# nooice98/HM16.9-NN_FME

Measured on AMD Instinct MI355X. Metric: sub-pel PU refinements/sec @ 1080p lowdelay_P QP22; bit-exact MV/SATD vs HM, higher is better.
Workload: dtype int16/int32 (NN f32)

## Files before the change

hm16.9-nn_fme_amd/csrc/fme_api.cpp:

```cpp
#include <dlfcn.h>
#include <hsa/hsa.h>
#include <hsa/hsa_ext_amd.h>

#include <chrono>
#include <cmath>
#include <cstdarg>
#include <cstdio>
#include <memory>

#include "fme_ctx.h"

using namespace fme;

namespace {
thread_local std::string g_last_error = "";
}


int fme::fail(int code, const char* fmt, ...) {
  char buf[512];
  va_list ap;
  va_start(ap, fmt);
  vsnprintf(buf, sizeof(buf), fmt, ap);
  va_end(ap);
  g_last_error = buf;
  return code;
}


extern "C" {

int fme_abi_version(void) { return FME_ABI_VERSION; }

const char* fme_last_error(void) { return g_last_error.c_str(); }

int fme_create(int device, const fme_config* cfg, fme_ctx** out_ctx) {
  if (!cfg || !out_ctx) return fail(FME_E_INVALID, "fme_create: null argument");
  *out_ctx = nullptr;
  if (cfg->bit_depth != 8 && cfg->bit_depth != 10)
    return fail(FME_E_UNSUPPORTED, "fme_create: bit_depth %d (8, or 10 for the main10 configurations)", cfg->bit_depth);
  if (cfg->nn_mode < 0 || cfg->nn_mode > 2) return fail(FME_E_INVALID, "fme_create: nn_mode %d", cfg->nn_mode);
  int ndev = 0;
  HIP_TRY(hipGetDeviceCount(&ndev));
  if (device < 0 || device >= ndev) return fail(FME_E_INVALID, "fme_create: device %d of %d", device, ndev);
  HIP_TRY(hipSetDevice(device));
  std::unique_ptr<fme_ctx> c(new fme_ctx());
  c->device = device;
  c->cfg = *cfg;
  HIP_TRY(c->d_pics.reserve(FME_MAX_PICTURES));
  HIP_TRY(c->d_mlambda.reserve(FME_MAX_LAMBDAS));
  HIP_TRY(c->d_nn.reserve(kNnPkFloats));
  HIP_TRY(c->counts.reserve(2 * kCountWords));
  HIP_TRY(hipMemset(c->counts.p, 0, 2 * kCountWords * sizeof(int32_t)));
  HIP_TRY(c->d_sched.reserve(1));
  c->sched_p = sched_params();
  {
    const char* m10 = std::getenv("FME_MAIN10_SEARCH");
    c->main10_px = m10 && std::strcmp(m10, "px") == 0;
  }
  HIP_TRY(hipEventCreateWithFlags(&c->ev_done, hipEventDisableTiming));
  HIP_TRY(c->nn_state.reserve(24));
  HIP_TRY(hipMemset(c->nn_state.p, 0, 24 * sizeof(uint32_t)));
  HIP_TRY(c->d_key_invalid.reserve(1));
  HIP_TRY(hipMemset(c->d_key_invalid.p, 0, sizeof(int32_t)));
  HIP_TRY(hipHostMalloc(reinterpret_cast<void**>(&c->h_counts), kCountWords * sizeof(int32_t), hipHostMallocDefault));
  if (cfg->max_jobs > 0) {
    const size_t n = (size_t)cfg->max_jobs;
    const size_t nb = (n + kJobsPerScanBlock - 1) / kJobsPerScanBlock;
    if (n * kNumClasses > (size_t)INT32_MAX) return fail(FME_E_INVALID, "fme_create: max_jobs %d", cfg->max_jobs);
    HIP_TRY(c->cls.reserve(n));
    HIP_TRY(c->perm.reserve(n * kNumClasses));
    HIP_TRY(c->blk_agg.reserve(nb * 9));
    HIP_TRY(c->blk_prefix.reserve(nb * 9));
  }
  *out_ctx = c.release();
  return FME_OK;
}

}
static int srv_stop(fme_ctx* c);
static void note_stream(fme_ctx* c, hipStream_t s) {
  for (int i = 0; i < c->n_used_streams; i++)
    if (c->used_streams[i] == s) return;
  if (c->n_used_streams < fme_ctx::kMaxStreams) c->used_streams[c->n_used_streams++] = s;
  else c->used_overflow = true;
}
static int drain_ctx(fme_ctx* c) {
  if (c->used_overflow) {
    HIP_TRY(hipDeviceSynchronize());
  } else {
    for (int i = 0; i < c->n_used_streams; i++) HIP_TRY(hipStreamSynchronize(c->used_streams[i]));
  }
  return FME_OK;
}
int fme::grow_keys(fme_ctx* c, size_t n) {
  if (n <= c->d_keys.cap) return FME_OK;
  FME_TRY(drain_ctx(c));
  HIP_TRY(c->d_keys.reserve(n));
  return FME_OK;
}
extern "C" {
int fme_destroy(fme_ctx* c) {
  if (!c) return FME_OK;
  (void)hipSetDevice(c->device);
  (void)srv_stop(c);
  (void)hipDeviceSynchronize();
  for (int i = 0; i < FME_MAX_PICTURES; i++)
    if (c->pic_owned[i] && c->pics[i].luma) (void)hipFree(const_cast<uint8_t*>(c->pics[i].luma));
  for (int i = 0; i < FME_MAX_PICTURES; i++)
    if (c->chroma_owned[i]) (void)hipFree(c->chroma_owned[i]);
  c->d_mc_jobs.release(); c->d_mc_planes.release(); c->d_mc_invalid.release(); c->d_mc_wp.release();
  c->d_tz_ext.release(); c->d_tz_sad.release(); c->d_tz_nn_in.release();
  c->d_amvp.release(); c->d_amvp_sad.release(); c->d_bikey.release(); c->d_key_invalid.release(); c->d_ch_i32.release(); c->d_tz_emi.release();
  c->h_pi_tasks.release(); c->h_pi_tsad.release(); c->h_pi_jobs.release(); c->h_pi_ext.release();
  c->h_pi_idx.release(); c->h_pi_psrc.release(); c->h_pi_mv.release(); c->h_pi_last.release();
  c->h_pi_ures.release(); c->h_pi_seq.release(); c->h_pi_rs.release(); c->h_pi_rows.release();
  c->d_pi_jobs.release(); c->d_pi_ext.release(); c->d_pi_idx.release();
  for (auto& e : c->ev_tz)
    if (e) (void)hipEventDestroy(e);
  for (auto& e : c->ev_mc)
    if (e) (void)hipEventDestroy(e);
  c->d_pe_tasks.release(); c->d_pe_dist.release(); c->d_pe_invalid.release();
  for (auto& e : c->ev_pe)
    if (e) (void)hipEventDestroy(e);
  c->d_sse_tasks.release(); c->d_sse_out.release(); c->d_sse_invalid.release();
  for (auto& e : c->ev_sse)
    if (e) (void)hipEventDestroy(e);
  c->d_surf_jobs.release(); c->d_surf_probe.release(); c->d_surf_out.release(); c->d_surf_pick.release();
  c->d_surf_invalid.release();
  for (auto& e : c->ev_surf)
    if (e) (void)hipEventDestroy(e);
  c->d_pics.release(); c->d_mlambda.release(); c->d_keys.release(); c->d_nn.release(); c->d_net.release();
  c->d_jobs.release(); c->d_res.release(); c->d_mv.release(); c->koff.release(); c->cls.release(); c->perm.release();
  c->counts.release(); c->blk_agg.release(); c->blk_prefix.release(); c->nn_state.release();
  c->d_sched.release();
  if (c->ev_done) (void)hipEventDestroy(c->ev_done);
  if (c->stage) (void)hipHostFree(c->stage);
  if (c->single_stream) (void)hipStreamDestroy(c->single_stream);
  if (c->box) (void)hipHostFree(c->box);
  if (c->srv_stream) (void)hipStreamDestroy(c->srv_stream);
  if (c->h_counts) (void)hipHostFree(c->h_counts);
  if (c->h_tab) (void)hipHostFree(c->h_tab);
  for (auto& e : c->tab_ev)
    if (e) (void)hipEventDestroy(e);
  for (auto& set : c->ev)
    for (auto& e : set)
      if (e) (void)hipEventDestroy(e);
  if (c->ev_fork) (void)hipEventDestroy(c->ev_fork);
  if (c->ev_join2) (void)hipEventDestroy(c->ev_join2);
  if (c->aux2) (void)hipStreamDestroy(c->aux2);
  if (c->ev_join) (void)hipEventDestroy(c->ev_join);
  if (c->aux) (void)hipStreamDestroy(c->aux);
  delete c;
  return FME_OK;
}

static void keep_chroma(fme_ctx* c, int id, int width, int height) {
  const PicDesc& o = c->pics[id];
  if (o.luma && o.width == width && o.height == height) return;
  if (c->chroma_owned[id]) (void)hipFree(c->chroma_owned[id]);
  c->chroma_owned[id] = nullptr;
  c->chroma_bytes[id] = 0;
  c->pics[id].cb = c->pics[id].cr = nullptr;
  c->pics[id].cstride = 0;
}

int fme_set_picture(fme_ctx* c, int id, const uint8_t* luma, int stride, int width, int height, void* stream) {
  if (!c || !luma) return fail(FME_E_INVALID, "fme_set_picture: null argument");
  if (id < 0 || id >= FME_MAX_PICTURES) return fail(FME_E_INVALID, "fme_set_picture: id %d", id);
  if (width <= 0 || height <= 0 || stride < width || width > 65535 || height > 65535)
    return fail(FME_E_INVALID, "fme_set_picture: %dx%d stride %d", width, height, stride);
  HIP_TRY(hipSetDevice(c->device));
  const size_t bps = c->cfg.bit_depth > 8 ? 2 : 1;
  const size_t bytes = (size_t)width * height * bps;
  uint8_t* dst = c->pic_owned[id] ? const_cast<uint8_t*>(c->pics[id].luma) : nullptr;
  if (!dst || c->pic_bytes[id] < bytes) {
    if (dst) HIP_TRY(hipFree(dst));
    dst = nullptr;
    HIP_TRY(hipMalloc(reinterpret_cast<void**>(&dst), bytes));
    c->pic_bytes[id] = bytes;
  }
  hipStream_t s = static_cast<hipStream_t>(stream);
  HIP_TRY(hipMemcpy2DAsync(dst, width * bps, luma, stride * bps, width * bps, height, hipMemcpyHostToDevice, s));
  HIP_TRY(hipStreamSynchronize(s));
  keep_chroma(c, id, width, height);
  c->pics[id] = PicDesc{dst, width, width, height, c->pics[id].cb, c->pics[id].cr, c->pics[id].cstride, 0};
  c->pic_owned[id] = true;
  c->tables_dirty = true;
  return FME_OK;
}

int fme_bind_picture_device(fme_ctx* c, int id, const uint8_t* d_luma, int stride, int width, int height) {
  if (!c || !d_luma) return fail(FME_E_INVALID, "fme_bind_picture_device: null argument");
  if (id < 0 || id >= FME_MAX_PICTURES) return fail(FME_E_INVALID, "fme_bind_picture_device: id %d", id);
  if (width <= 0 || height <= 0 || stride < width) return fail(FME_E_INVALID, "fme_bind_picture_device: geometry");
  HIP_TRY(hipSetDevice(c->device));
  if (c->pic_owned[id] && c->pics[id].luma) HIP_TRY(hipFree(const_cast<uint8_t*>(c->pics[id].luma)));
  c->pic_owned[id] = false;
  c->pic_bytes[id] = 0;
  keep_chroma(c, id, width, height);
  c->pics[id] = PicDesc{d_luma, stride, width, height, c->pics[id].cb, c->pics[id].cr, c->pics[id].cstride, 0};
  c->tables_dirty = true;
  return FME_OK;
}

int fme_set_picture_chroma(fme_ctx* c, int id, const uint8_t* cb, const uint8_t* cr, int stride, void* stream) {
  if (!c || !cb || !cr) return fail(FME_E_INVALID, "fme_set_picture_chroma: null argument");
  if (id < 0 || id >= FME_MAX_PICTURES) return fail(FME_E_INVALID, "fme_set_picture_chroma: id %d", id);
  if (!c->pics[id].luma) return fail(FME_E_STATE, "fme_set_picture_chroma: picture %d has no luma plane", id);
  const int cw = c->pics[id].width >> 1, ch = c->pics[id].height >> 1;
  if (stride < cw) return fail(FME_E_INVALID, "fme_set_picture_chroma: stride %d < %d", stride, cw);
  HIP_TRY(hipSetDevice(c->device));
  const size_t bps = c->cfg.bit_depth > 8 ? 2 : 1;
  const size_t bytes = 2 * (size_t)cw * ch * bps;
  if (!c->chroma_owned[id] || c->chroma_bytes[id] < bytes) {
    if (c->chroma_owned[id]) HIP_TRY(hipFree(c->chroma_owned[id]));
    c->chroma_owned[id] = nullptr;
    HIP_TRY(hipMalloc(reinterpret_cast<void**>(&c->chroma_owned[id]), bytes));
    c->chroma_bytes[id] = bytes;
  }
  uint8_t* dcb = c->chroma_owned[id];
  uint8_t* dcr = dcb + (size_t)cw * ch * bps;
  hipStream_t s = static_cast<hipStream_t>(stream);
  HIP_TRY(hipMemcpy2DAsync(dcb, cw * bps, cb, stride * bps, cw * bps, ch, hipMemcpyHostToDevice, s));
  HIP_TRY(hipMemcpy2DAsync(dcr, cw * bps, cr, stride * bps, cw * bps, ch, hipMemcpyHostToDevice, s));
  HIP_TRY(hipStreamSynchronize(s));
  c->pics[id].cb = dcb;
  c->pics[id].cr = dcr;
  c->pics[id].cstride = cw;
  c->tables_dirty = true;
  return FME_OK;
}

int fme_bind_picture_chroma_device(fme_ctx* c, int id, const uint8_t* d_cb, const uint8_t* d_cr, int stride) {
  if (!c || !d_cb || !d_cr) return fail(FME_E_INVALID, "fme_bind_picture_chroma_device: null argument");
  if (id < 0 || id >= FME_MAX_PICTURES) return fail(FME_E_INVALID, "fme_bind_picture_chroma_device: id %d", id);
  if (!c->pics[id].luma) return fail(FME_E_STATE, "fme_bind_picture_chroma_device: picture %d has no luma plane", id);
  if (stride < (c->pics[id].width >> 1)) return fail(FME_E_INVALID, "fme_bind_picture_chroma_device: stride %d", stride);
  HIP_TRY(hipSetDevice(c->device));
  if (c->chroma_owned[id]) HIP_TRY(hipFree(c->chroma_owned[id]));
  c->chroma_owned[id] = nullptr;
  c->chroma_bytes[id] = 0;
  c->pics[id].cb = d_cb;
  c->pics[id].cr = d_cr;
  c->pics[id].cstride = stride;
  c->tables_dirty = true;
  return FME_OK;
}

int fme_set_lambda(fme_ctx* c, int id, double lambda) {
  if (!c || id < 0 || id >= FME_MAX_LAMBDAS || !(lambda >= 0.0)) return fail(FME_E_INVALID, "fme_set_lambda: bad argument");
  const double sq = std::sqrt(lambda);
  c->mlambda[id] = 65536.0 * sq + 0;
  c->lambda_set[id] = true;
  c->tables_dirty = true;
  return FME_OK;
}

int fme_set_motion_lambda(fme_ctx* c, int id, double ml) {
  if (!c || id < 0 || id >= FME_MAX_LAMBDAS || !(ml >= 0.0)) return fail(FME_E_INVALID, "fme_set_motion_lambda: bad argument");
  c->mlambda[id] = ml;
  c->lambda_set[id] = true;
  c->tables_dirty = true;
  return FME_OK;
}

int fme_set_keys(fme_ctx* c, const int16_t* keys, size_t count, void* stream) {
  if (!c || (!keys && count)) return fail(FME_E_INVALID, "fme_set_keys: null argument");
  HIP_TRY(hipSetDevice(c->device));
  FME_TRY(srv_stop(c));
  FME_TRY(grow_keys(c, count));
  hipStream_t s = static_cast<hipStream_t>(stream);
  if (count) HIP_TRY(hipMemcpyAsync(c->d_keys.p, keys, count * sizeof(int16_t), hipMemcpyHostToDevice, s));
  HIP_TRY(hipMemsetAsync(c->d_key_invalid.p, 0, sizeof(int32_t), s));
  HIP_TRY(hipStreamSynchronize(s));
  c->n_keys = count;
  return FME_OK;
}

int fme_load_nn_weights(fme_ctx* c, const float* params, int count) {
  if (!c || !params) return fail(FME_E_INVALID, "fme_load_nn_weights: null argument");
  if (count != FME_NN_PARAMS) return fail(FME_E_INVALID, "fme_load_nn_weights: %d params, expected %d", count, FME_NN_PARAMS);
  HIP_TRY(hipSetDevice(c->device));
  std::vector<float> packed(kNnPkFloats);
  nn_pack(params, packed.data());
  HIP_TRY(hipMemcpy(c->d_nn.p, packed.data(), kNnPkFloats * sizeof(float), hipMemcpyHostToDevice));
  c->nn_loaded = true;
  c->nn_gen++;
  return FME_OK;
}

int fme_nn_param_count(const fme_nn_net* n) {
  if (!n) return fail(FME_E_INVALID, "fme_nn_param_count: null descriptor");
  if (n->n_hidden < 1 || n->n_hidden > FME_NN_MAX_HIDDEN)
    return fail(FME_E_INVALID, "fme_nn_param_count: n_hidden %d", n->n_hidden);
  if (n->precision != FME_NN_F32 && n->precision != FME_NN_F64)
    return fail(FME_E_INVALID, "fme_nn_param_count: precision %d", n->precision);
  if (n->embedding < FME_NN_EMB_NONE || n->embedding > FME_NN_EMB_SWAP)
    return fail(FME_E_INVALID, "fme_nn_param_count: embedding %d", n->embedding);
  if (n->out_act != FME_NN_OUT_LINEAR && n->out_act != FME_NN_OUT_SIGMOID)
    return fail(FME_E_INVALID, "fme_nn_param_count: out_act %d", n->out_act);
  if (n->carry_hidden >> n->n_hidden) return fail(FME_E_INVALID, "fme_nn_param_count: carry_hidden 0x%x", n->carry_hidden);
  if (n->input_flags & ~(FME_NN_IN_SLOT_RESET | FME_NN_IN_TZ_RING))
    return fail(FME_E_INVALID, "fme_nn_param_count: input_flags 0x%x", n->input_flags);
  if ((n->input_flags & FME_NN_IN_TZ_RING) && ((n->input_flags & FME_NN_IN_SLOT_RESET) || n->carry_hidden))
    return fail(FME_E_INVALID, "fme_nn_param_count: FME_NN_IN_TZ_RING with FME_NN_IN_SLOT_RESET or carry_hidden");
  int count = n->embedding ? 64 : 0, fan = n->embedding ? 17 : 9;
  for (int l = 0; l < n->n_hidden; l++) {
    const int w = n->width[l];
    if (w < 1 || w > FME_NN_MAX_WIDTH) return fail(FME_E_INVALID, "fme_nn_param_count: width[%d] = %d", l, w);
    count += w * fan + 3 * w;
    fan = w;
  }
  return count + 49 * fan + 49 + 27;
}

int fme_load_nn_net(fme_ctx* c, const fme_nn_net* n, const double* params, int count) {
  if (!c || !n || !params) return fail(FME_E_INVALID, "fme_load_nn_net: null argument");
  const int need = fme_nn_param_count(n);
  if (need < 0) return need;
  if (count != need) return fail(FME_E_INVALID, "fme_load_nn_net: %d params, the descriptor needs %d", count, need);
  if (n->carry_hidden)
    return fail(FME_E_UNSUPPORTED, "fme_load_nn_net: carry_hidden 0x%x (hidden layers carried across calls) is not "
                "supported by the batch engines", n->carry_hidden);
  HIP_TRY(hipSetDevice(c->device));
  const size_t bytes = nn_deep_packed_bytes(*n);
  if (!bytes) return fail(FME_E_UNSUPPORTED, "fme_load_nn_net: no kernel for this net");
  std::vector<unsigned char> packed(bytes);
  nn_deep_pack(*n, params, packed.data());
  FME_TRY(drain_ctx(c));
  HIP_TRY(c->d_net.reserve(bytes));
  HIP_TRY(hipMemcpy(c->d_net.p, packed.data(), bytes, hipMemcpyHostToDevice));
  c->net = *n;
  c->net_loaded = true;
  return FME_OK;
}

int fme_set_nn_engine(fme_ctx* c, int engine) {
  if (!c || (engine != FME_NN_ENGINE_EXACT && engine != FME_NN_ENGINE_MFMA))
    return fail(FME_E_INVALID, "fme_set_nn_engine: bad argument");
  c->nn_engine = engine;
  return FME_OK;
}

int fme_set_nn_logit_output(fme_ctx* c, void* d_logits, int capacity) {
  if (!c) return fail(FME_E_INVALID, "fme_set_nn_logit_output: null ctx");
  if (d_logits && capacity <= 0) return fail(FME_E_INVALID, "fme_set_nn_logit_output: capacity %d", capacity);
  c->nn_logits = capacity > 0 ? d_logits : nullptr;
  c->nn_logits_cap = d_logits ? capacity : 0;
  return FME_OK;
}

int fme_set_nn_inputs(fme_ctx* c, const uint32_t* d_rows, int capacity) {
  if (!c) return fail(FME_E_INVALID, "fme_set_nn_inputs: null ctx");
  if (d_rows && capacity <= 0) return fail(FME_E_INVALID, "fme_set_nn_inputs: capacity %d", capacity);
  c->nn_in = capacity > 0 ? d_rows : nullptr;
  c->nn_in_cap = d_rows ? capacity : 0;
  return FME_OK;
}

int fme_set_nn_margin_output(fme_ctx* c, float* d_margin, int capacity) {
  if (!c) return fail(FME_E_INVALID, "fme_set_nn_margin_output: null ctx");
  if (d_margin && capacity <= 0) return fail(FME_E_INVALID, "fme_set_nn_margin_output: capacity %d", capacity);
  c->nn_margin = capacity > 0 ? d_margin : nullptr;
  c->nn_margin_cap = d_margin ? capacity : 0;
  return FME_OK;
}

int fme_nn_reset_state(fme_ctx* c) {
  if (!c) return fail(FME_E_INVALID, "fme_nn_reset_state: null ctx");
  for (uint32_t& v : c->pending_state) v = 0;
  c->state_pending = true;
  return FME_OK;
}

int fme_nn_get_state(fme_ctx* c, uint32_t* out12) {
  if (!c || !out12) return fail(FME_E_INVALID, "fme_nn_get_state: null argument");
  if (c->state_pending) {
    std::memcpy(out12, c->pending_state, sizeof(c->pending_state));
    return FME_OK;
  }
  HIP_TRY(hipSetDevice(c->device));
  FME_TRY(drain_ctx(c));
  HIP_TRY(hipMemcpy(out12, c->nn_state.p + 12 * c->state_cur, 12 * sizeof(uint32_t), hipMemcpyDeviceToHost));
  return FME_OK;
}

int fme_nn_set_state(fme_ctx* c, const uint32_t* in12) {
  if (!c || !in12) return fail(FME_E_INVALID, "fme_nn_set_state: null argument");
  std::memcpy(c->pending_state, in12, sizeof(c->pending_state));
  c->state_pending = true;
  return FME_OK;
}

int fme_nn_copy_state_device(fme_ctx* c, uint32_t* d_out12, void* stream) {
  if (!c || !d_out12) return fail(FME_E_INVALID, "fme_nn_copy_state_device: null argument");
  HIP_TRY(hipSetDevice(c->device));
  hipStream_t s = static_cast<hipStream_t>(stream);
  if (c->state_pending)
    HIP_TRY(launch_put_state(d_out12, c->pending_state, s));
  else
    HIP_TRY(hipMemcpyAsync(d_out12, c->nn_state.p + 12 * c->state_cur, 12 * sizeof(uint32_t),
                           hipMemcpyDeviceToDevice, s));
  return FME_OK;
}

}

static int ensure_work(fme_ctx* c, int n) {
  const size_t nb = ((size_t)n + kJobsPerScanBlock - 1) / kJobsPerScanBlock;
  if ((size_t)n * kNumClasses > (size_t)INT32_MAX) return fail(FME_E_INVALID, "%d jobs in one batch", n);
  HIP_TRY(c->cls.reserve(n));
  HIP_TRY(c->perm.reserve((size_t)n * kNumClasses));
  HIP_TRY(c->blk_agg.reserve(nb * 9));
  HIP_TRY(c->blk_prefix.reserve(nb * 9));
  HIP_TRY(c->koff.reserve(n));
  return FME_OK;
}

static int counts_begin(fme_ctx* c, hipStream_t s) {
  if (c->counts_dirty) HIP_TRY(hipMemsetAsync(c->counts.p, 0, 2 * kCountWords * sizeof(int32_t), s));
  c->counts_dirty = true;
  return FME_OK;
}
static void counts_done(fme_ctx* c) {
  c->counts_cur ^= 1;
  c->counts_dirty = false;
}

static WorkBufs work_bufs(fme_ctx* c) {
  WorkBufs w{};
  w.cls = c->cls.p;
  w.perm = c->perm.p;
  w.perm_cap = (int32_t)(c->perm.cap / kNumClasses);
  w.koff = c->koff.p;
  w.counts = c->counts.p + c->counts_cur * kCountWords;
  w.counts_next = c->counts.p + (c->counts_cur ^ 1) * kCountWords;
  w.cursor = w.counts + kCursorWord;
  w.tile_ctr = w.counts + kTileCtrWord;
  w.blk_agg = c->blk_agg.p;
  w.blk_prefix = c->blk_prefix.p;
  w.nn_state = c->nn_state.p;
  w.sched = c->d_sched.p;
  w.mv_out = nullptr;
  return w;
}

BatchArgs fme::batch_args(const fme_ctx* c, const fme_job* jobs, int n) {
  BatchArgs a{};
  a.jobs = jobs;
  a.keys = c->d_keys.p;
  a.n_keys = (int64_t)c->n_keys;
  a.key_invalid = c->d_key_invalid.p;
  a.mlambda = c->d_mlambda.p;
  a.pics = c->d_pics.p;
  a.n = n;
  a.use_hadamard = c->cfg.use_hadamard ? 1 : 0;
  a.fen = c->cfg.fast_inter_mode;
  return a;
}

int fme::sync_tables(fme_ctx* c, hipStream_t s) {
  note_stream(c, s);
  FME_TRY(srv_stop(c));
  if (!c->tables_dirty) return FME_OK;
  if (!c->h_tab) {
    void* p = nullptr;
    HIP_TRY(hipHostMalloc(&p, fme_ctx::kTabSlots * sizeof(TablesSlot), hipHostMallocMapped));
    c->h_tab = static_cast<TablesSlot*>(p);
    void* d = nullptr;
    HIP_TRY(hipHostGetDevicePointer(&d, p, 0));
    c->h_tab_dev = static_cast<TablesSlot*>(d);
    for (auto& e : c->tab_ev) HIP_TRY(hipEventCreateWithFlags(&e, hipEventDisableTiming));
  }
  const int k = c->tab_next;
  c->tab_next = (k + 1) % fme_ctx::kTabSlots;
  if (c->tab_used[k]) HIP_TRY(hipEventSynchronize(c->tab_ev[k]));
  std::memcpy(c->h_tab[k].pics, c->pics, sizeof(c->pics));
  std::memcpy(c->h_tab[k].ml, c->mlambda, sizeof(c->mlambda));
  HIP_TRY(launch_put_tables(c->d_pics.p, c->d_mlambda.p, c->h_tab_dev + k, s));
  HIP_TRY(hipEventRecord(c->tab_ev[k], s));
  c->tab_used[k] = true;
  c->tables_dirty = false;
  return FME_OK;
}

static int apply_pending_state(fme_ctx* c, hipStream_t s) {
  if (!c->state_pending) return FME_OK;
  HIP_TRY(launch_put_state(c->nn_state.p + 12 * c->state_cur, c->pending_state, s));
  c->state_pending = false;
  return FME_OK;
}

static int harvest_events(fme_ctx* c, bool wait_all) {
  while (c->ev_tail != c->ev_head) {
    const int b = c->ev_tail % fme_ctx::kEvSets;
    hipEvent_t* e = c->ev[b];
    if (wait_all) {
      HIP_TRY(hipEventSynchronize(e[6]));
    } else {
      const hipError_t q = hipEventQuery(e[6]);
      if (q == hipErrorNotReady) break;
      HIP_TRY(q);
    }
    float* ms = c->last_ms;
    HIP_TRY(hipEventElapsedTime(&ms[0], e[0], e[3]));
    ms[1] = 0.f;
    HIP_TRY(hipEventElapsedTime(&ms[2], e[3], e[5]));
    HIP_TRY(hipEventElapsedTime(&ms[3], e[5], e[6]));
    HIP_TRY(hipEventElapsedTime(&ms[4], e[0], e[6]));
    HIP_TRY(hipEventElapsedTime(&ms[5], e[3], e[4]));
    ms[6] = 0.f;
    for (int i = 0; i < FME_NUM_TIMINGS; i++) c->acc_ms[i] += ms[i];
    c->acc_batches++;
    c->timed = true;
    c->ev_tail++;
  }
  return FME_OK;
}

int fme::refine_batch(fme_ctx* c, const fme_job* d_jobs, fme_result* d_res, fme_mv_result* d_mv, int n,
                      hipStream_t s, const fme_job_packed* d_pjobs, const int32_t* d_key_base) {
  if (c->cfg.nn_mode == 1 && !c->nn_loaded) return fail(FME_E_STATE, "fme_refine_device: nn_mode set but no weights loaded");
  if (c->cfg.nn_mode == 2 && !c->net_loaded) return fail(FME_E_STATE, "fme_refine_device: nn_mode 2 but no net loaded");
  if (c->cfg.nn_mode == 2 && c->nn_margin && n > c->nn_margin_cap)
    return fail(FME_E_INVALID, "fme_refine: %d jobs but the margin output holds %d", n, c->nn_margin_cap);
  if (c->cfg.nn_mode == 2 && c->nn_logits && n > c->nn_logits_cap)
    return fail(FME_E_INVALID, "fme_refine: %d jobs but the logit output holds %d", n, c->nn_logits_cap);
  HIP_TRY(hipSetDevice(c->device));
  FME_TRY(ensure_work(c, n));
  FME_TRY(sync_tables(c, s));
  FME_TRY(apply_pending_state(c, s));

  BatchArgs a = batch_args(c, d_jobs, n);
  a.pjobs = d_jobs ? nullptr : d_pjobs;
  a.key_base = d_key_base;
  a.koff = c->koff.p;
  a.res = d_res;
  a.nn_mode = c->cfg.nn_mode ? 1 : 0;
  a.nn_in = c->nn_in;
  a.nn_in_cap = c->nn_in_cap;
  WorkBufs w = work_bufs(c);
  w.mv_out = d_mv;

  const bool prof = c->profiling;
  hipEvent_t* ev = nullptr;
  int eb = 0;
  if (prof) {
    FME_TRY(harvest_events(c, false));
    if (c->ev_head - c->ev_tail == fme_ctx::kEvSets) {
      HIP_TRY(hipEventSynchronize(c->ev[c->ev_tail % fme_ctx::kEvSets][6]));
      FME_TRY(harvest_events(c, false));
    }
    eb = c->ev_head % fme_ctx::kEvSets;
    ev = c->ev[eb];
    HIP_TRY(hipEventRecord(ev[0], s));
  }
  FME_TRY(counts_begin(c, s));
  HIP_TRY(launch_front(a, w, c->sched_p, s));
  if (prof) HIP_TRY(hipEventRecord(ev[3], s));
  if (c->ev_search) HIP_TRY(hipEventRecord(c->ev_search, s));
  if (c->cfg.bit_depth > 8) {
    if (c->main10_px)
      HIP_TRY(launch_search_px(a, w, c->cfg.bit_depth, s, nullptr));
    else
      HIP_TRY(launch_search_lane10(a, w, s));
  } else {
    HIP_TRY(launch_search_lane(a, w, c->search_reserve, s));
  }
  if (prof) HIP_TRY(hipEventRecord(ev[4], s));
  if (prof) HIP_TRY(hipEventRecord(ev[5], s));
  HIP_TRY(c->cfg.nn_mode == 2
              ? launch_nn_deep_tail(c->net, c->d_net.p, c->nn_margin, c->nn_logits, a, w, c->state_cur, c->nn_engine, s)
              : launch_nn_tail(a, w, c->d_nn.p, c->state_cur, s));
  if (prof) {
    HIP_TRY(hipEventRecord(ev[6], s));
    c->ev_head++;
  }
  HIP_TRY(hipEventRecord(c->ev_done, s));
  counts_done(c);
  c->batch_issued = true;
  if (a.nn_mode) c->state_cur ^= 1;
  return FME_OK;
}

int fme::check_rejected(fme_ctx* c, hipStream_t s, const char* name, const char* what) {
  HIP_TRY(hipMemcpyAsync(c->h_counts, &c->d_sched.p->invalid, sizeof(int32_t), hipMemcpyDeviceToHost, s));
  HIP_TRY(hipStreamSynchronize(s));
  if (c->h_counts[0] > 0)
    return fail(FME_E_INVALID, "%s: %d job(s) %s", name, c->h_counts[0], what);
  return FME_OK;
}

extern "C" {

int fme_refine_device(fme_ctx* c, const fme_job* d_jobs, fme_result* d_res, int n, void* stream) {
  if (!c || (n > 0 && (!d_jobs || !d_res))) return fail(FME_E_INVALID, "fme_refine_device: null argument");
  if (n < 0) return fail(FME_E_INVALID, "fme_refine_device: n = %d", n);
  if (n == 0) return FME_OK;
  return refine_batch(c, d_jobs, d_res, nullptr, n, static_cast<hipStream_t>(stream));
}

int fme_refine_mv_device(fme_ctx* c, const fme_job* d_jobs, fme_mv_result* d_out, int n, void* stream) {
  if (!c || (n > 0 && (!d_jobs || !d_out))) return fail(FME_E_INVALID, "fme_refine_mv_device: null argument");
  if (n < 0) return fail(FME_E_INVALID, "fme_refine_mv_device: n = %d", n);
  if (n == 0) return FME_OK;
  HIP_TRY(hipSetDevice(c->device));
  HIP_TRY(c->d_res.reserve(n));
  return refine_batch(c, d_jobs, c->d_res.p, d_out, n, static_cast<hipStream_t>(stream));
}

int fme_pack_jobs(const fme_job* jobs, int n, fme_job_packed* out, int32_t* key_base) {
  if (n < 0 || (n > 0 && (!jobs || !out || !key_base))) return fail(FME_E_INVALID, "fme_pack_jobs: bad argument");
  const int waves = (n + FME_PACK_WAVE - 1) / FME_PACK_WAVE;
  for (int wv = 0; wv < waves; wv++) {
    int64_t next = -1;
    key_base[wv] = -1;
    const int e = std::min(n, (wv + 1) * FME_PACK_WAVE);
    for (int i = wv * FME_PACK_WAVE; i < e; i++) {
      const fme_job& j = jobs[i];
      const char* why = nullptr;
      if ((j.x & 3) || (j.y & 3) || (j.w & 3) || (j.h & 3) || j.w < 4 || j.w > 64 || j.h < 4 || j.h > 64)
        why = "PU off the 4x4 grid or not 4..64";
      else if (j.x >= 8192 || j.y >= 8192) why = "x or y >= 8192";
      else if (j.org_id >= 64 || j.ref_id >= 64 || j.lambda_id >= 32) why = "slot id >= 64 or lambda_id >= 32";
      else if (j.flags & ~15u) why = "unknown flags";
      else if (j.bits_in >= 64) why = "bits_in >= 64";
      else if (j.mv_x <= -32767 || j.mv_x >= 32766 || j.mv_y <= -32767 || j.mv_y >= 32766) why = "int16-extreme mv";
      else if (j.key_offset >= 0) {
        if (next < 0) key_base[wv] = j.key_offset;
        else if ((int64_t)j.key_offset != next) why = "key block not dense in job order within its wave";
        next = (int64_t)j.key_offset + (int64_t)j.w * j.h;
      }
      if (why) return fail(FME_E_UNSUPPORTED, "fme_pack_jobs: job %d: %s (use fme_job)", i, why);
      uint32_t rg = 0;
      if (j.mv_y - 1 >= j.lt_y) rg |= FME_PK_RANGE_TOP;
      if (j.mv_y + 1 <= j.rb_y) rg |= FME_PK_RANGE_BOTTOM;
      if (j.mv_x - 1 >= j.lt_x) rg |= FME_PK_RANGE_LEFT;
      if (j.mv_x + 1 <= j.rb_x) rg |= FME_PK_RANGE_RIGHT;
      fme_job_packed p;
      p.pu = (uint32_t)(j.x >> 2) | ((uint32_t)(j.y >> 2) << 11) | ((uint32_t)((j.w >> 2) - 1) << 22) |
             ((uint32_t)((j.h >> 2) - 1) << 26);
      p.ctl = (uint32_t)j.org_id | ((uint32_t)j.ref_id << 6) | ((uint32_t)j.lambda_id << 12) |
              ((uint32_t)j.flags << 17) | ((uint32_t)(j.key_offset >= 0) << 21) | (rg << 22) |
              ((uint32_t)j.bits_in << 26);
      p.mv_x = j.mv_x;
      p.mv_y = j.mv_y;
      p.mvp_x = j.mvp_x;
      p.mvp_y = j.mvp_y;
      out[i] = p;
    }
  }
  return FME_OK;
}

int fme_unpack_jobs(const fme_job_packed* packed, const int32_t* key_base, int n, fme_job* out) {
  if (n < 0 || (n > 0 && (!packed || !key_base || !out))) return fail(FME_E_INVALID, "fme_unpack_jobs: bad argument");
  int64_t next = 0;
  for (int i = 0; i < n; i++) {
    const fme_job_packed& p = packed[i];
    if (i % FME_PACK_WAVE == 0) next = key_base[i / FME_PACK_WAVE];
    fme_job j;
    j.x = (uint16_t)((p.pu & 2047u) * 4u);
    j.y = (uint16_t)(((p.pu >> 11) & 2047u) * 4u);
    j.w = (uint8_t)((((p.pu >> 22) & 15u) + 1u) * 4u);
    j.h = (uint8_t)((((p.pu >> 26) & 15u) + 1u) * 4u);
    j.org_id = (uint8_t)(p.ctl & 63u);
    j.ref_id = (uint8_t)((p.ctl >> 6) & 63u);
    j.lambda_id = (uint8_t)((p.ctl >> 12) & 31u);
    j.flags = (uint8_t)((p.ctl >> 17) & 15u);
    const uint32_t rg = (p.ctl >> 22) & 15u;
    j.bits_in = (uint16_t)(p.ctl >> 26);
    j.mv_x = p.mv_x;
    j.mv_y = p.mv_y;
    j.mvp_x = p.mvp_x;
    j.mvp_y = p.mvp_y;
    j.lt_x = (int16_t)(p.mv_x - ((rg & FME_PK_RANGE_LEFT) ? 1 : 0));
    j.rb_x = (int16_t)(p.mv_x + ((rg & FME_PK_RANGE_RIGHT) ? 1 : 0));
    j.lt_y = (int16_t)(p.mv_y - ((rg & FME_PK_RANGE_TOP) ? 1 : 0));
    j.rb_y = (int16_t)(p.mv_y + ((rg & FME_PK_RANGE_BOTTOM) ? 1 : 0));
    if ((p.ctl >> 21) & 1u) {
      j.key_offset = (int32_t)next;
      next += (int64_t)j.w * j.h;
    } else {
      j.key_offset = -1;
    }
    out[i] = j;
  }
  return FME_OK;
}

static int refine_packed(fme_ctx* c, const fme_job_packed* d_jobs, const int32_t* d_key_base, fme_result* d_res,
                         fme_mv_result* d_mv, int n, void* stream, const char* fn) {
  if (!c || (n > 0 && (!d_jobs || !d_key_base || !(d_res || d_mv)))) return fail(FME_E_INVALID, "%s: null argument", fn);
  if (n < 0) return fail(FME_E_INVALID, "%s: n = %d", fn, n);
  if (n == 0) return FME_OK;
  HIP_TRY(hipSetDevice(c->device));
  if (!d_res) {
    HIP_TRY(c->d_res.reserve(n));
    d_res = c->d_res.p;
  }
  return refine_batch(c, nullptr, d_res, d_mv, n, static_cast<hipStream_t>(stream), d_jobs, d_key_base);
}

int fme_refine_packed_device(fme_ctx* c, const fme_job_packed* d_jobs, const int32_t* d_key_base, fme_result* d_res,
                             int n, void* stream) {
  if (c && n > 0 && !d_res) return fail(FME_E_INVALID, "fme_refine_packed_device: null argument");
  return refine_packed(c, d_jobs, d_key_base, d_res, nullptr, n, stream, "fme_refine_packed_device");
}

int fme_refine_mv_packed_device(fme_ctx* c, const fme_job_packed* d_jobs, const int32_t* d_key_base,
                                fme_mv_result* d_out, int n, void* stream) {
  if (c && n > 0 && !d_out) return fail(FME_E_INVALID, "fme_refine_mv_packed_device: null argument");
  return refine_packed(c, d_jobs, d_key_base, nullptr, d_out, n, stream, "fme_refine_mv_packed_device");
}

int fme_set_search_event(fme_ctx* c, void* event) {
  if (!c) return fail(FME_E_INVALID, "fme_set_search_event: null ctx");
  c->ev_search = static_cast<hipEvent_t>(event);
  return FME_OK;
}

int fme_set_search_reserve(fme_ctx* c, int workgroups) {
  if (!c || workgroups < 0 || workgroups > 4096) return fail(FME_E_INVALID, "fme_set_search_reserve: bad argument");
  c->search_reserve = workgroups;
  return FME_OK;
}

int fme_download_device(fme_ctx* c, const void* d_src, void* h_dst, size_t bytes, int workgroups, void* stream) {
  if (!c || (bytes && (!d_src || !h_dst))) return fail(FME_E_INVALID, "fme_download_device: null argument");
  if ((bytes & 15) || (reinterpret_cast<uintptr_t>(d_src) & 15) || (reinterpret_cast<uintptr_t>(h_dst) & 15))
    return fail(FME_E_INVALID, "fme_download_device: pointers and size must be 16-byte multiples");
  if (workgroups < 0 || workgroups > 1024) return fail(FME_E_INVALID, "fme_download_device: %d workgroups", workgroups);
  if (!bytes) return FME_OK;
  HIP_TRY(hipSetDevice(c->device));
  void* dst = nullptr;
  if (hipHostGetDevicePointer(&dst, h_dst, 0) != hipSuccess || !dst) {
    (void)hipGetLastError();
    return fail(FME_E_INVALID, "fme_download_device: h_dst is not pinned host memory");
  }
  HIP_TRY(launch_download(d_src, dst, bytes / 16, workgroups ? workgroups : 8, static_cast<hipStream_t>(stream)));
  return FME_OK;
}

namespace {
struct HsaCopyApi {
  hsa_status_t (*iterate_agents)(hsa_status_t (*)(hsa_agent_t, void*), void*);
  hsa_status_t (*agent_get_info)(hsa_agent_t, hsa_agent_info_t, void*);
  hsa_status_t (*signal_create)(hsa_signal_value_t, uint32_t, const hsa_agent_t*, hsa_signal_t*);
  hsa_status_t (*signal_destroy)(hsa_signal_t);
  hsa_signal_value_t (*signal_wait)(hsa_signal_t, hsa_signal_condition_t, hsa_signal_value_t, uint64_t,
                                    hsa_wait_state_t);
  hsa_status_t (*copy_on_engine)(void*, hsa_agent_t, const void*, hsa_agent_t, size_t, uint32_t,
                                 const hsa_signal_t*, hsa_signal_t, hsa_amd_sdma_engine_id_t, bool);
};
bool hsa_copy_api(HsaCopyApi& a) {
  void* h = dlopen("libhsa-runtime64.so.1", RTLD_LAZY | RTLD_NOLOAD);
  if (!h) h = dlopen("libhsa-runtime64.so.1", RTLD_LAZY);
  if (!h) return false;
  a.iterate_agents = reinterpret_cast<decltype(a.iterate_agents)>(dlsym(h, "hsa_iterate_agents"));
  a.agent_get_info = reinterpret_cast<decltype(a.agent_get_info)>(dlsym(h, "hsa_agent_get_info"));
  a.signal_create = reinterpret_cast<decltype(a.signal_create)>(dlsym(h, "hsa_signal_create"));
  a.signal_destroy = reinterpret_cast<decltype(a.signal_destroy)>(dlsym(h, "hsa_signal_destroy"));
  a.signal_wait = reinterpret_cast<decltype(a.signal_wait)>(dlsym(h, "hsa_signal_wait_scacquire"));
  a.copy_on_engine = reinterpret_cast<decltype(a.copy_on_engine)>(dlsym(h, "hsa_amd_memory_async_copy_on_engine"));
  return a.iterate_agents && a.agent_get_info && a.signal_create && a.signal_destroy && a.signal_wait &&
         a.copy_on_engine;
}
struct AgentPick {
  const HsaCopyApi* api;
  uint32_t bdf, domain;
  bool have_gpu = false, have_cpu = false;
  hsa_agent_t gpu{}, cpu{};
};
hsa_status_t pick_agent(hsa_agent_t ag, void* data) {
  AgentPick* p = static_cast<AgentPick*>(data);
  hsa_device_type_t t;
  if (p->api->agent_get_info(ag, HSA_AGENT_INFO_DEVICE, &t) != HSA_STATUS_SUCCESS) return HSA_STATUS_SUCCESS;
  if (t == HSA_DEVICE_TYPE_CPU && !p->have_cpu) {
    p->cpu = ag;
    p->have_cpu = true;
  } else if (t == HSA_DEVICE_TYPE_GPU && !p->have_gpu) {
    uint32_t bdf = 0, dom = 0;
    p->api->agent_get_info(ag, static_cast<hsa_agent_info_t>(HSA_AMD_AGENT_INFO_BDFID), &bdf);
    p->api->agent_get_info(ag, static_cast<hsa_agent_info_t>(HSA_AMD_AGENT_INFO_DOMAIN), &dom);
    if (bdf == p->bdf && dom == p->domain) {
      p->gpu = ag;
      p->have_gpu = true;
    }
  }
  return HSA_STATUS_SUCCESS;
}
}

int fme_warm_copy_engines(fme_ctx* c, int* engines) {
  if (!c) return fail(FME_E_INVALID, "fme_warm_copy_engines: null ctx");
  if (engines) *engines = 0;
  HIP_TRY(hipSetDevice(c->device));
  HsaCopyApi api{};
  if (!hsa_copy_api(api)) return fail(FME_E_DEVICE, "fme_warm_copy_engines: HSA runtime symbols not found");
  int bus = 0, dev = 0, dom = 0;
  HIP_TRY(hipDeviceGetAttribute(&bus, hipDeviceAttributePciBusId, c->device));
  HIP_TRY(hipDeviceGetAttribute(&dev, hipDeviceAttributePciDeviceId, c->device));
  HIP_TRY(hipDeviceGetAttribute(&dom, hipDeviceAttributePciDomainID, c->device));
  AgentPick pk{&api, (uint32_t)((bus << 8) | (dev << 3)), (uint32_t)dom};
  api.iterate_agents(pick_agent, &pk);
  if (!pk.have_gpu || !pk.have_cpu) return fail(FME_E_DEVICE, "fme_warm_copy_engines: HSA agents not found");
  uint32_t n_sdma = 0, n_xgmi = 0;
  api.agent_get_info(pk.gpu, static_cast<hsa_agent_info_t>(HSA_AMD_AGENT_INFO_NUM_SDMA_ENG), &n_sdma);
  api.agent_get_info(pk.gpu, static_cast<hsa_agent_info_t>(HSA_AMD_AGENT_INFO_NUM_SDMA_XGMI_ENG), &n_xgmi);
  const int n_eng = std::min(16, (int)(n_sdma + n_xgmi));
  constexpr size_t kBytes = 4096;
  void* d = nullptr;
  void* h = nullptr;
  HIP_TRY(hipMalloc(&d, kBytes));
  if (hipHostMalloc(&h, kBytes, hipHostMallocDefault) != hipSuccess) {
    (void)hipFree(d);
    return fail(FME_E_NOMEM, "fme_warm_copy_engines: host buffer");
  }
  std::memset(h, 0, kBytes);
  int warmed = 0;
  for (int e = 0; e < n_eng; e++) {
    bool ok = true;
    for (int dir = 0; dir < 2 && ok; dir++) {
      hsa_signal_t sig;
      if (api.signal_create(1, 0, nullptr, &sig) != HSA_STATUS_SUCCESS) {
        ok = false;
        break;
      }
      const auto eid = static_cast<hsa_amd_sdma_engine_id_t>(1u << e);
      const hsa_status_t st = dir == 0 ? api.copy_on_engine(d, pk.gpu, h, pk.cpu, kBytes, 0, nullptr, sig, eid, true)
                                       : api.copy_on_engine(h, pk.cpu, d, pk.gpu, kBytes, 0, nullptr, sig, eid, true);
      if (st == HSA_STATUS_SUCCESS)
        api.signal_wait(sig, HSA_SIGNAL_CONDITION_LT, 1, UINT64_MAX, HSA_WAIT_STATE_BLOCKED);
      else
        ok = false;
      api.signal_destroy(sig);
    }
    warmed += ok ? 1 : 0;
  }
  (void)hipHostFree(h);
  (void)hipFree(d);
  if (engines) *engines = warmed;
  return FME_OK;
}

int fme_refine_status(fme_ctx* c) {
  if (!c) return fail(FME_E_INVALID, "fme_refine_status: null ctx");
  if (!c->batch_issued) return 0;
  HIP_TRY(hipSetDevice(c->device));
  HIP_TRY(hipEventSynchronize(c->ev_done));
  int32_t v = 0;
  HIP_TRY(hipMemcpy(&v, &c->d_sched.p->invalid, sizeof(v), hipMemcpyDeviceToHost));
  return v;
}

int fme_debug_front(fme_ctx* c, int32_t* perm_out, long long perm_words, int32_t* sched_out, int sched_words,
                    int32_t* cap_out) {
  if (!c || !c->batch_issued) return fail(FME_E_STATE, "fme_debug_front: no batch issued");
  if (perm_words < 0 || (size_t)perm_words > c->perm.cap || sched_words < 0 ||
      (size_t)sched_words * sizeof(int32_t) > sizeof(Schedule))
    return fail(FME_E_INVALID, "fme_debug_front: length");
  HIP_TRY(hipSetDevice(c->device));
  HIP_TRY(hipEventSynchronize(c->ev_done));
  if (perm_out && perm_words) HIP_TRY(hipMemcpy(perm_out, c->perm.p, (size_t)perm_words * sizeof(int32_t), hipMemcpyDeviceToHost));
  if (sched_out && sched_words) HIP_TRY(hipMemcpy(sched_out, c->d_sched.p, (size_t)sched_words * sizeof(int32_t), hipMemcpyDeviceToHost));
  if (cap_out) *cap_out = (int32_t)(c->perm.cap / kNumClasses);
  return FME_OK;
}

}

int fme::tz_run(fme_ctx* c, fme_job* d_jobs, const fme_tz_ext* d_ext, uint32_t* d_sad, int n, void* stream,
                int16_t* d_emi, uint32_t* d_nn_in, int ext_stride) {
  if (!c || (n > 0 && (!d_jobs || !d_ext))) return fail(FME_E_INVALID, "fme_integer_search_device: null argument");
  if (n < 0) return fail(FME_E_INVALID, "fme_integer_search_device: n = %d", n);
  if (n == 0) return FME_OK;
  HIP_TRY(hipSetDevice(c->device));
  hipStream_t s = static_cast<hipStream_t>(stream);
  FME_TRY(ensure_work(c, n));
  FME_TRY(sync_tables(c, s));
  BatchArgs a = batch_args(c, d_jobs, n);
  a.nn_in = c->nn_in;
  a.nn_in_cap = c->nn_in_cap;
  WorkBufs w = work_bufs(c);
  if (c->profiling) {
    if (!c->ev_tz[0]) {
      HIP_TRY(hipEventCreate(&c->ev_tz[0]));
      HIP_TRY(hipEventCreate(&c->ev_tz[1]));
    }
  }
  c->counts_dirty = true;
  HIP_TRY(hipMemsetAsync(w.counts, 0, kCountWords * sizeof(int32_t), s));
  HIP_TRY(launch_classify(a, w, s));
  HIP_TRY(hipMemcpyAsync(c->h_counts, w.counts, kCountWords * sizeof(int32_t), hipMemcpyDeviceToHost, s));
  HIP_TRY(hipStreamSynchronize(s));
  if (c->h_counts[kNumClasses] > 0)
    return fail(FME_E_INVALID, "fme_integer_search_device: %d job(s) with an unsupported PU size or unset picture/lambda/key",
                c->h_counts[kNumClasses]);
  const bool keyed = c->h_counts[kKeyedWord] > 0;
  TzSchedule sc{};
  int off = 0, nb[3] = {0, 0, 0};
  for (int k = 0; k < kNumClasses; k++) {
    const int cnt = c->h_counts[k];
    sc.class_off[k] = off;
    sc.class_cnt[k] = cnt;
    for (int q = 0; q < 3; q++) sc.prefix[q][k] = nb[q];
    nb[tz_kernel_of(k)] += cnt;
    off += cnt;
  }
  for (int q = 0; q < 3; q++) sc.prefix[q][kNumClasses] = nb[q];
  HIP_TRY(launch_scatter(a, w, c->sched_p, s));
  TzArgs ta{};
  ta.a = a;
  ta.perm = c->perm.p;
  ta.jobs_out = d_jobs;
  ta.ext = d_ext;
  ta.ext_stride = ext_stride;
  ta.sad = d_sad;
  ta.emi_mv = d_emi;
  ta.nn_in = d_nn_in;
  if (c->profiling) HIP_TRY(hipEventRecord(c->ev_tz[0], s));
  if (!c->aux) HIP_TRY(hipStreamCreateWithFlags(&c->aux, hipStreamNonBlocking));
  if (!c->aux2) HIP_TRY(hipStreamCreateWithFlags(&c->aux2, hipStreamNonBlocking));
  if (!c->ev_fork) HIP_TRY(hipEventCreateWithFlags(&c->ev_fork, hipEventDisableTiming));
  if (!c->ev_join) HIP_TRY(hipEventCreateWithFlags(&c->ev_join, hipEventDisableTiming));
  if (!c->ev_join2) HIP_TRY(hipEventCreateWithFlags(&c->ev_join2, hipEventDisableTiming));
  int cw = 0, ch = 0, npic = 0;
  for (int i = 0; i < FME_MAX_PICTURES; i++)
    if (c->pics[i].luma) {
      cw = std::max(cw, (c->pics[i].width + 63) / 64);
      ch = std::max(ch, (c->pics[i].height + 63) / 64);
      npic = i + 1;
    }
  const long long np = (long long)npic * cw * ch;
  const bool stage = c->cfg.bit_depth == 8 || std::getenv("FME_TZ10_UNSTAGED") == nullptr;
  if (FME_TZ_STAGE && stage && np > 0 && np <= (1LL << 20)) {
    const size_t words = 8 + 12 * (size_t)np;
    if (c->d_tzp.cap < words || c->d_tzp_perm.cap < (size_t)n) {
      FME_TRY(drain_ctx(c));
      HIP_TRY(c->d_tzp.reserve(words));
      HIP_TRY(c->d_tzp_perm.reserve(n));
    }
    TzPairs tp{};
    int32_t* b = c->d_tzp.p;
    tp.nseg = b;
    tp.cnt = b + 8;
    tp.cursor = tp.cnt + 3 * np;
    tp.off = tp.cursor + 3 * np;
    tp.seg = tp.off + 3 * np;
    tp.perm = c->d_tzp_perm.p;
    tp.np = (int32_t)np;
    tp.cw = cw;
    tp.ch = ch;
    HIP_TRY(hipMemsetAsync(b, 0, (8 + 3 * (size_t)np) * sizeof(int32_t), s));
    HIP_TRY(launch_tz_pairs(ta, tp, w.cls, n, s));
    HIP_TRY(hipEventRecord(c->ev_fork, s));
    HIP_TRY(hipStreamWaitEvent(c->aux, c->ev_fork, 0));
    HIP_TRY(hipStreamWaitEvent(c->aux2, c->ev_fork, 0));
    HIP_TRY(launch_tz_staged(ta, tp, 0, keyed, c->cfg.bit_depth, c->aux));
    HIP_TRY(launch_tz_staged(ta, tp, 1, keyed, c->cfg.bit_depth, c->aux2));
    HIP_TRY(launch_tz_staged(ta, tp, 2, keyed, c->cfg.bit_depth, s));
  } else {
    HIP_TRY(hipEventRecord(c->ev_fork, s));
    HIP_TRY(hipStreamWaitEvent(c->aux, c->ev_fork, 0));
    HIP_TRY(hipStreamWaitEvent(c->aux2, c->ev_fork, 0));
    HIP_TRY(launch_tz_wave(ta, sc, 0, keyed, c->cfg.bit_depth, c->aux));
    HIP_TRY(launch_tz_wave(ta, sc, 1, keyed, c->cfg.bit_depth, c->aux2));
    HIP_TRY(launch_tz_wave(ta, sc, 2, keyed, c->cfg.bit_depth, s));
  }
  HIP_TRY(hipEventRecord(c->ev_join, c->aux));
  HIP_TRY(hipEventRecord(c->ev_join2, c->aux2));
  HIP_TRY(hipStreamWaitEvent(s, c->ev_join, 0));
  HIP_TRY(hipStreamWaitEvent(s, c->ev_join2, 0));
  if (c->profiling) HIP_TRY(hipEventRecord(c->ev_tz[1], s));
  c->tz_timed = c->profiling;
  return FME_OK;
}

static int tz_run_host(fme_ctx* c, fme_job* jobs, const fme_tz_ext* ext, uint32_t* sad, int n, void* stream,
                       int16_t* emi, uint32_t* nn_in = nullptr, int ext_stride = (int)sizeof(fme_tz_ext)) {
  if (!c || (n > 0 && (!jobs || !ext))) return fail(FME_E_INVALID, "fme_integer_search: null argument");
  if (n <= 0) return n == 0 ? FME_OK : fail(FME_E_INVALID, "fme_integer_search: n = %d", n);
  HIP_TRY(hipSetDevice(c->device));
  hipStream_t s = static_cast<hipStream_t>(stream);
  HIP_TRY(c->d_jobs.reserve(n));
  HIP_TRY(c->d_tz_ext.reserve(((size_t)n * ext_stride + sizeof(fme_tz_ext) - 1) / sizeof(fme_tz_ext)));
  HIP_TRY(c->d_tz_sad.reserve(n));
  if (emi) HIP_TRY(c->d_tz_emi.reserve((size_t)2 * n));
  if (nn_in) HIP_TRY(c->d_tz_nn_in.reserve((size_t)9 * n));
  HIP_TRY(hipMemcpyAsync(c->d_jobs.p, jobs, (size_t)n * sizeof(fme_job), hipMemcpyHostToDevice, s));
  HIP_TRY(hipMemcpyAsync(c->d_tz_ext.p, ext, (size_t)n * ext_stride, hipMemcpyHostToDevice, s));
  if (nn_in) HIP_TRY(hipMemcpyAsync(c->d_tz_nn_in.p, nn_in, (size_t)9 * n * sizeof(uint32_t), hipMemcpyHostToDevice, s));
  int rc = tz_run(c, c->d_jobs.p, c->d_tz_ext.p, c->d_tz_sad.p, n, stream, emi ? c->d_tz_emi.p : nullptr,
                  nn_in ? c->d_tz_nn_in.p : nullptr, ext_stride);
  if (rc) return rc;
  HIP_TRY(hipMemcpyAsync(jobs, c->d_jobs.p, (size_t)n * sizeof(fme_job), hipMemcpyDeviceToHost, s));
  if (sad) HIP_TRY(hipMemcpyAsync(sad, c->d_tz_sad.p, (size_t)n * sizeof(uint32_t), hipMemcpyDeviceToHost, s));
  if (emi) HIP_TRY(hipMemcpyAsync(emi, c->d_tz_emi.p, (size_t)n * 2 * sizeof(int16_t), hipMemcpyDeviceToHost, s));
  if (nn_in) HIP_TRY(hipMemcpyAsync(nn_in, c->d_tz_nn_in.p, (size_t)9 * n * sizeof(uint32_t), hipMemcpyDeviceToHost, s));
  HIP_TRY(hipStreamSynchronize(s));
  return FME_OK;
}

extern "C" {

int fme_integer_search_device(fme_ctx* c, fme_job* d_jobs, const fme_tz_ext* d_ext, uint32_t* d_sad, int n,
                              void* stream) {
  return tz_run(c, d_jobs, d_ext, d_sad, n, stream, nullptr);
}

int fme_integer_search(fme_ctx* c, fme_job* jobs, const fme_tz_ext* ext, uint32_t* sad, int n, void* stream) {
  return tz_run_host(c, jobs, ext, sad, n, stream, nullptr);
}

int fme_integer_search2_device(fme_ctx* c, fme_job* d_jobs, const fme_tz_ext2* d_ext, uint32_t* d_sad, int n,
                               void* stream) {
  return tz_run(c, d_jobs, reinterpret_cast<const fme_tz_ext*>(d_ext), d_sad, n, stream, nullptr, nullptr,
                (int)sizeof(fme_tz_ext2));
}

int fme_integer_search2(fme_ctx* c, fme_job* jobs, const fme_tz_ext2* ext, uint32_t* sad, int n, void* stream) {
  return tz_run_host(c, jobs, reinterpret_cast<const fme_tz_ext*>(ext), sad, n, stream, nullptr, nullptr,
                     (int)sizeof(fme_tz_ext2));
}

int fme_integer_search_ring_device(fme_ctx* c, fme_job* d_jobs, const fme_tz_ext* d_ext, uint32_t* d_sad,
                                   uint32_t* d_nn_in, int n, void* stream) {
  if (!d_nn_in && n > 0) return fail(FME_E_INVALID, "fme_integer_search_ring_device: null nn_in");
  return tz_run(c, d_jobs, d_ext, d_sad, n, stream, nullptr, d_nn_in);
}

int fme_integer_search_ring(fme_ctx* c, fme_job* jobs, const fme_tz_ext* ext, uint32_t* sad, uint32_t* nn_in,
                            int n, void* stream) {
  if (!nn_in && n > 0) return fail(FME_E_INVALID, "fme_integer_search_ring: null nn_in");
  return tz_run_host(c, jobs, ext, sad, n, stream, nullptr, nn_in);
}

int fme_integer_search_last_ms(fme_ctx* c, float* ms) {
  if (!c || !ms) return fail(FME_E_INVALID, "fme_integer_search_last_ms: null argument");
  if (!c->tz_timed) return fail(FME_E_STATE, "fme_integer_search_last_ms: no profiled integer search");
  HIP_TRY(hipEventSynchronize(c->ev_tz[1]));
  HIP_TRY(hipEventElapsedTime(ms, c->ev_tz[0], c->ev_tz[1]));
  return FME_OK;
}

static int refine_host(fme_ctx* c, const fme_job* jobs, fme_result* res, fme_mv_result* mv, int n, void* stream,
                       const char* name) {
  if (!c || (n > 0 && (!jobs || (!res && !mv)))) return fail(FME_E_INVALID, "%s: null argument", name);
  if (n <= 0) return n == 0 ? FME_OK : fail(FME_E_INVALID, "%s: n = %d", name, n);
  HIP_TRY(hipSetDevice(c->device));
  hipStream_t s = static_cast<hipStream_t>(stream);
  HIP_TRY(c->d_jobs.reserve(n));
  HIP_TRY(c->d_res.reserve(n));
  if (mv) HIP_TRY(c->d_mv.reserve(n));
  HIP_TRY(hipMemcpyAsync(c->d_jobs.p, jobs, (size_t)n * sizeof(fme_job), hipMemcpyHostToDevice, s));
  FME_TRY(refine_batch(c, c->d_jobs.p, c->d_res.p, mv ? c->d_mv.p : nullptr, n, s));
  if (mv)
    HIP_TRY(hipMemcpyAsync(mv, c->d_mv.p, (size_t)n * sizeof(fme_mv_result), hipMemcpyDeviceToHost, s));
  else
    HIP_TRY(hipMemcpyAsync(res, c->d_res.p, (size_t)n * sizeof(fme_result), hipMemcpyDeviceToHost, s));
  return check_rejected(c, s, name, "with an unsupported PU size or unset picture/lambda/key");
}

int fme_refine(fme_ctx* c, const fme_job* jobs, fme_result* res, int n, void* stream) {
  return refine_host(c, jobs, res, nullptr, n, stream, "fme_refine");
}

int fme_refine_mv(fme_ctx* c, const fme_job* jobs, fme_mv_result* out, int n, void* stream) {
  return refine_host(c, jobs, nullptr, out, n, stream, "fme_refine_mv");
}

static int ensure_stage(fme_ctx* c) {
  if (c->stage) return FME_OK;
  void* p = nullptr;
  HIP_TRY(hipHostMalloc(&p, sizeof(SingleStage), hipHostMallocMapped));
  c->stage = static_cast<SingleStage*>(p);
  void* d = nullptr;
  HIP_TRY(hipHostGetDevicePointer(&d, p, 0));
  c->stage_dev = static_cast<uint8_t*>(d);
  HIP_TRY(hipStreamCreateWithFlags(&c->single_stream, hipStreamNonBlocking));
  std::memset(c->stage, 0, sizeof(SingleStage));
  return FME_OK;
}

static int class_of(int w, int h) {
  for (int k = 0; k < kNumClasses; k++)
    if (kClassW[k] == w && kClassH[k] == h) return k;
  return -1;
}

static int single_wait(fme_ctx* c, uint32_t seq) {
  volatile uint32_t* f = &c->stage->flag;
  for (long it = 1; *f != seq; it++) {
    __builtin_ia32_pause();
    if ((it & 1023) == 0) {
      const hipError_t q = hipStreamQuery(c->single_stream);
      if (q != hipErrorNotReady && *f != seq) {
        if (q != hipSuccess) return fail(FME_E_DEVICE, "single-PU kernel: %s", hipGetErrorString(q));
        return fail(FME_E_DEVICE, "single-PU kernel ended without its completion word");
      }
    }
  }
  __atomic_thread_fence(__ATOMIC_ACQUIRE);
  return FME_OK;
}

constexpr uint64_t kSrvIdleUs = 2000;
constexpr uint64_t kSrvLifeMs = 100;

static int srv_open(fme_ctx* c) {
  if (c->box) return FME_OK;
  void* p = nullptr;
  HIP_TRY(hipHostMalloc(&p, sizeof(SrvBox), hipHostMallocMapped));
  std::memset(p, 0, sizeof(SrvBox));
  c->box = static_cast<SrvBox*>(p);
  void* d = nullptr;
  HIP_TRY(hipHostGetDevicePointer(&d, p, 0));
  c->box_dev = static_cast<SrvBox*>(d);
  HIP_TRY(hipStreamCreateWithFlags(&c->srv_stream, hipStreamNonBlocking));
  int khz = 0;
  if (hipDeviceGetAttribute(&khz, hipDeviceAttributeWallClockRate, c->device) == hipSuccess && khz > 0)
    c->srv_khz = (uint64_t)khz;
  return FME_OK;
}

static int srv_launch(fme_ctx* c) {
  if (c->srv_orphan) {
    const hipError_t q = hipStreamQuery(c->srv_stream);
    if (q == hipErrorNotReady)
      return fail(FME_E_DEVICE, "single-call server: the instance that timed out is still running");
    (void)hipGetLastError();
    c->srv_orphan = false;
  }
  __atomic_store_n(&c->box->req[0][3], 0u, __ATOMIC_RELEASE);
  const uint32_t epoch = ++c->srv_epoch;
  c->srv_nn_gen = c->nn_gen;
  HIP_TRY(launch_server(c->box_dev, c->nn_loaded ? c->d_nn.p : nullptr, c->srv_done, epoch,
                        kSrvIdleUs * c->srv_khz / 1000, kSrvLifeMs * c->srv_khz, c->cfg.bit_depth, c->srv_stream));
  c->srv_running = true;
  return FME_OK;
}

constexpr double kSrvWaitLimitS = 2.0;
static bool srv_waited_too_long(std::chrono::steady_clock::time_point t0) {
  return std::chrono::duration<double>(std::chrono::steady_clock::now() - t0).count() > kSrvWaitLimitS;
}

static int srv_join(fme_ctx* c) {
  volatile uint32_t* st = &c->box->stopped;
  const auto t0 = std::chrono::steady_clock::now();
  for (long it = 1; *st != c->srv_epoch; it++) {
    __builtin_ia32_pause();
    if ((it & 1023) == 0) {
      const hipError_t q = hipStreamQuery(c->srv_stream);
      if (q != hipErrorNotReady && *st != c->srv_epoch) {
        c->srv_running = false;
        if (q != hipSuccess) return fail(FME_E_DEVICE, "single-call server: %s", hipGetErrorString(q));
        return fail(FME_E_DEVICE, "single-call server ended without its stop word");
      }
      if (srv_waited_too_long(t0)) {
        c->srv_running = false;
        c->srv_orphan = true;
        return fail(FME_E_DEVICE, "single-call server: no stop word after %.1f s", kSrvWaitLimitS);
      }
    }
  }
  c->srv_running = false;
  HIP_TRY(hipStreamSynchronize(c->srv_stream));
  return FME_OK;
}

static int srv_stop(fme_ctx* c) {
  if (!c->srv_running) return FME_OK;
  __atomic_store_n(&c->box->req[0][3], 1u, __ATOMIC_RELEASE);
  return srv_join(c);
}

static int srv_call(fme_ctx* c, bool uses_nn) {
  int rc = FME_OK;
  if (c->srv_running && uses_nn && c->srv_nn_gen != c->nn_gen) rc = srv_stop(c);
  if (!rc && !c->srv_running) rc = srv_launch(c);
  if (rc) return rc;
  const uint32_t seq = c->srv_done + 1;
  __atomic_store_n(&c->box->req[0][0], seq, __ATOMIC_RELEASE);
  volatile uint32_t* done = &c->box->res[0];
  volatile uint32_t* st = &c->box->stopped;
  const auto t0 = std::chrono::steady_clock::now();
  for (long it = 1; *done != seq; it++) {
    __builtin_ia32_pause();
    if (*st == c->srv_epoch && *done != seq) {
      c->srv_running = false;
      HIP_TRY(hipStreamSynchronize(c->srv_stream));
      if (srv_waited_too_long(t0))
        return fail(FME_E_DEVICE, "single-call server: call %u unanswered after %.1f s", seq, kSrvWaitLimitS);
      FME_TRY(srv_launch(c));
    } else if ((it & 4095) == 0) {
      const hipError_t q = hipStreamQuery(c->srv_stream);
      if (q != hipErrorNotReady && q != hipSuccess) {
        c->srv_running = false;
        return fail(FME_E_DEVICE, "single-call server: %s", hipGetErrorString(q));
      }
      if (srv_waited_too_long(t0)) {
        __atomic_store_n(&c->box->req[0][3], 1u, __ATOMIC_RELEASE);
        if (srv_join(c) != FME_OK) c->srv_orphan = true;
        c->srv_running = false;
        return fail(FME_E_DEVICE, "single-call server: call %u unanswered after %.1f s", seq, kSrvWaitLimitS);
      }
    }
  }
  __atomic_thread_fence(__ATOMIC_ACQUIRE);
  c->srv_done = seq;
  return FME_OK;
}

int fme_frac_dif_single(fme_ctx* c, int lossless, const int16_t* key, int key_stride, int w, int h,
                        const int16_t* ref, int ref_stride, int mv_int_x, int mv_int_y, int mvp_x,
                        int mvp_y, double motion_lambda, int16_t* half_xy, int16_t* qtr_xy,
                        uint32_t* cost) {
  if (!c || !key || !ref || !half_xy || !qtr_xy || !cost) return fail(FME_E_INVALID, "fme_frac_dif_single: null argument");
  const int cls = class_of(w, h);
  if (cls < 0) return fail(FME_E_UNSUPPORTED, "fme_frac_dif_single: %dx%d", w, h);
  const int px = mvp_x - 4 * mv_int_x, py = mvp_y - 4 * mv_int_y;
  if (px < -32768 || px > 32767 || py < -32768 || py > 32767) return fail(FME_E_INVALID, "fme_frac_dif_single: predictor out of range");
  HIP_TRY(hipSetDevice(c->device));
  FME_TRY(srv_open(c));
  SrvBox* b = c->box;
  srv_pack_frac(b, c->srv_done + 1, c->cfg.bit_depth, lossless || !c->cfg.use_hadamard, c->srv_marks, key, key_stride, w,
                h, ref, ref_stride, mv_int_x, mv_int_y, px, py, motion_lambda);
  FME_TRY(srv_call(c, false));
  const uint32_t hq = b->res[2];
  half_xy[0] = (int16_t)(int8_t)(hq & 0xFF);
  half_xy[1] = (int16_t)(int8_t)((hq >> 8) & 0xFF);
  qtr_xy[0] = (int16_t)(int8_t)((hq >> 16) & 0xFF);
  qtr_xy[1] = (int16_t)(int8_t)(hq >> 24);
  *cost = b->res[1];
  return FME_OK;
}

int fme_nn_pred_single(fme_ctx* c, const uint32_t* e, uint32_t cc, int pu_h, int pu_w, int* nn_class, int16_t* out4) {
  if (!c || !e || !nn_class) return fail(FME_E_INVALID, "fme_nn_pred_single: null argument");
  const bool deep = c->cfg.nn_mode == 2;
  if (deep ? !c->net_loaded : !c->nn_loaded) return fail(FME_E_STATE, "fme_nn_pred_single: no weights loaded");
  HIP_TRY(hipSetDevice(c->device));
  int rc;
  if (!deep) {
    FME_TRY(srv_open(c));
    const uint32_t in[12] = {e[0], e[1], e[2], e[3], e[4], e[5], e[6], e[7], cc, (uint32_t)pu_h, (uint32_t)pu_w, 0u};
    const uint32_t seq = c->srv_done + 1;
    for (int b = 1; b < 5; b++) {
      for (int k = 0; k < 3; k++) c->box->req[b][1 + k] = in[3 * (b - 1) + k];
      __atomic_store_n(&c->box->req[b][0], seq, __ATOMIC_RELEASE);
    }
    c->box->req[0][1] = kSrvNn | (c->srv_marks ? (uint32_t)kSrvMarks : 0u);
    FME_TRY(srv_call(c, true));
    *nn_class = (int)c->box->res[1];
  } else {
  rc = srv_stop(c);
  if (!rc) rc = ensure_stage(c);
  if (rc) return rc;
  NnIn11 in{};
  for (int s = 0; s < 8; s++) in.v[s] = e[s];
  in.v[8] = cc;
  in.v[9] = (uint32_t)pu_h;
  in.v[10] = (uint32_t)pu_w;
  int32_t* d_out = reinterpret_cast<int32_t*>(c->stage_dev + offsetof(SingleStage, nn_out));
  uint32_t* d_flag = reinterpret_cast<uint32_t*>(c->stage_dev + offsetof(SingleStage, flag));
  const uint32_t seq = ++c->single_seq;
  HIP_TRY(launch_nn_deep_single(c->net, c->d_net.p, in, d_out, d_flag, seq, c->single_stream));
  FME_TRY(single_wait(c, seq));
  *nn_class = c->stage->nn_out[0];
  }
  const int cls = *nn_class;
  if (out4) {
    const int ox = cls % 7 - 3, oy = cls / 7 - 3;
    auto split = [](int o, int16_t& hf, int16_t& qt) {
      static const int8_t H[7] = {-1, -1, 0, 0, 0, 1, 1}, Q[7] = {-1, 0, -1, 0, 1, 0, 1};
      hf = H[o + 3];
      qt = Q[o + 3];
    };
    split(ox, out4[0], out4[1]);
    split(oy, out4[2], out4[3]);
  }
  return FME_OK;
}

int fme_single_last_device_us(fme_ctx* c, float* us, int count) {
  if (!c || (count > 0 && !us)) return fail(FME_E_INVALID, "fme_single_last_device_us: null argument");
  const double k = 1000.0 / (double)c->srv_khz;
  if (count > 1) c->srv_marks = true;
  for (int i = 0; i < count && i < 5; i++)
    us[i] = !c->box ? 0.0f : (float)((double)(i == 0 ? c->box->res[3] : c->box->marks[i - 1]) * k);
  return FME_OK;
}

int fme_search_kernel_of_shape(int width, int height) {
  for (int k = 0; k < kNumClasses; k++)
    if (kClassW[k] == width && kClassH[k] == height) {
      return 0;
    }
  return -1;
}

static const char* mc_job_problem(const fme_ctx* c, const fme_mc_job& j, int width, int height) {
  if (j.w < 4 || j.h < 4 || j.w > 64 || j.h > 64 || (j.w & 3) || (j.h & 3)) return "PU size";
  if (!(j.flags & (FME_MC_L0 | FME_MC_L1)) || (j.flags & ~(FME_MC_L0 | FME_MC_L1 | FME_MC_WP))) return "list flags";
  if ((int)j.x + j.w > width || (int)j.y + j.h > height) return "PU outside the picture";
  for (int l = 0; l < 2; l++) {
    if (!(j.flags & (1u << l))) continue;
    if (j.ref_id[l] >= FME_MAX_PICTURES) return "reference id";
    const PicDesc& p = c->pics[j.ref_id[l]];
    if (!p.luma || !p.cb || !p.cr) return "reference picture without luma + chroma";
    if (p.width != width || p.height != height) return "reference picture dimensions";
  }
  return nullptr;
}

static int mc_launch(fme_ctx* c, const fme_mc_job* d_jobs, int n, uint8_t* y, int ys, uint8_t* cb, uint8_t* cr,
                     int cs, int width, int height, hipStream_t s) {
  HIP_TRY(c->d_mc_invalid.reserve(1));
  HIP_TRY(hipMemsetAsync(c->d_mc_invalid.p, 0, sizeof(int32_t), s));
  if (int e = sync_tables(c, s)) return e;
  if (!c->wp_init) {
    for (auto& l : c->h_wp)
      for (auto& p : l)
        for (auto& q : p) q = fme_wp_param{1, 0, 0, {0, 0, 0}};
    c->wp_init = true;
  }
  if (c->wp_dirty) {
    HIP_TRY(c->d_mc_wp.reserve(sizeof(c->h_wp) / sizeof(fme_wp_param)));
    HIP_TRY(hipMemcpyAsync(c->d_mc_wp.p, c->h_wp, sizeof(c->h_wp), hipMemcpyHostToDevice, s));
    c->wp_dirty = false;
  }
  McArgs a{};
  a.wp = c->d_mc_wp.p;
  a.jobs = d_jobs;
  a.pics = c->d_pics.p;
  a.y = y;
  a.cb = cb;
  a.cr = cr;
  a.invalid = c->d_mc_invalid.p;
  a.n = n;
  a.y_stride = ys;
  a.c_stride = cs;
  a.width = width;
  a.height = height;
  a.bit_depth = c->cfg.bit_depth;
  if (c->profiling) {
    if (!c->ev_mc[0]) {
      HIP_TRY(hipEventCreate(&c->ev_mc[0]));
      HIP_TRY(hipEventCreate(&c->ev_mc[1]));
    }
    HIP_TRY(hipEventRecord(c->ev_mc[0], s));
  }
  HIP_TRY(launch_mc(a, s));
  if (c->profiling) HIP_TRY(hipEventRecord(c->ev_mc[1], s));
  c->mc_timed = c->profiling;
  return FME_OK;
}

static int mc_check_planes(const void* y, int ys, const void* cb, const void* cr, int cs, int width, int height) {
  if (!y || !cb || !cr) return fail(FME_E_INVALID, "motion compensation: null plane");
  if (width <= 0 || height <= 0 || (width & 1) || (height & 1) || ys < width || cs < width / 2)
    return fail(FME_E_INVALID, "motion compensation: geometry %dx%d strides %d/%d", width, height, ys, cs);
  return FME_OK;
}

int fme_motion_compensate(fme_ctx* c, const fme_mc_job* jobs, int n, uint8_t* y, int ys, uint8_t* cb, uint8_t* cr,
                          int cs, int width, int height, void* stream) {
  if (!c || (n > 0 && !jobs) || n < 0) return fail(FME_E_INVALID, "fme_motion_compensate: bad argument");
  if (int e = mc_check_planes(y, ys, cb, cr, cs, width, height)) return e;
  for (int i = 0; i < n; i++)
    if (const char* why = mc_job_problem(c, jobs[i], width, height))
      return fail(FME_E_INVALID, "fme_motion_compensate: job %d: %s", i, why);
  if (n == 0) return FME_OK;
  HIP_TRY(hipSetDevice(c->device));
  hipStream_t s = static_cast<hipStream_t>(stream);
  const size_t bps = c->cfg.bit_depth > 8 ? 2 : 1;
  const size_t ly = (size_t)width * height * bps, lc = ly / 4;
  HIP_TRY(c->d_mc_jobs.reserve(n));
  HIP_TRY(c->d_mc_planes.reserve(ly + 2 * lc));
  uint8_t* dy = c->d_mc_planes.p;
  uint8_t* dcb = dy + ly;
  uint8_t* dcr = dcb + lc;
  const int cw = width / 2, ch = height / 2;
  HIP_TRY(hipMemcpyAsync(c->d_mc_jobs.p, jobs, n * sizeof(fme_mc_job), hipMemcpyHostToDevice, s));
  HIP_TRY(hipMemcpy2DAsync(dy, width * bps, y, ys * bps, width * bps, height, hipMemcpyHostToDevice, s));
  HIP_TRY(hipMemcpy2DAsync(dcb, cw * bps, cb, cs * bps, cw * bps, ch, hipMemcpyHostToDevice, s));
  HIP_TRY(hipMemcpy2DAsync(dcr, cw * bps, cr, cs * bps, cw * bps, ch, hipMemcpyHostToDevice, s));
  if (int e = mc_launch(c, c->d_mc_jobs.p, n, dy, width, dcb, dcr, cw, width, height, s)) return e;
  HIP_TRY(hipMemcpy2DAsync(y, ys * bps, dy, width * bps, width * bps, height, hipMemcpyDeviceToHost, s));
  HIP_TRY(hipMemcpy2DAsync(cb, cs * bps, dcb, cw * bps, cw * bps, ch, hipMemcpyDeviceToHost, s));
  HIP_TRY(hipMemcpy2DAsync(cr, cs * bps, dcr, cw * bps, cw * bps, ch, hipMemcpyDeviceToHost, s));
  HIP_TRY(hipStreamSynchronize(s));
  return FME_OK;
}

int fme_motion_compensate_device(fme_ctx* c, const fme_mc_job* d_jobs, int n, uint8_t* d_y, int ys, uint8_t* d_cb,
                                 uint8_t* d_cr, int cs, int width, int height, void* stream) {
  if (!c || (n > 0 && !d_jobs) || n < 0) return fail(FME_E_INVALID, "fme_motion_compensate_device: bad argument");
  if (int e = mc_check_planes(d_y, ys, d_cb, d_cr, cs, width, height)) return e;
  HIP_TRY(hipSetDevice(c->device));
  return mc_launch(c, d_jobs, n, d_y, ys, d_cb, d_cr, cs, width, height, static_cast<hipStream_t>(stream));
}

int fme_mc_invalid_count(fme_ctx* c) {
  if (!c) return fail(FME_E_INVALID, "fme_mc_invalid_count: null ctx");
  if (!c->d_mc_invalid.p) return 0;
  HIP_TRY(hipSetDevice(c->device));
  int32_t v = 0;
  FME_TRY(drain_ctx(c));
  HIP_TRY(hipMemcpy(&v, c->d_mc_invalid.p, sizeof(v), hipMemcpyDeviceToHost));
  return v;
}

int fme_set_wp(fme_ctx* c, int list, int ref_id, const fme_wp_param* p) {
  if (!c || !p) return fail(FME_E_INVALID, "fme_set_wp: null argument");
  if (list < 0 || list > 1 || ref_id < 0 || ref_id >= FME_MAX_PICTURES)
    return fail(FME_E_INVALID, "fme_set_wp: list %d reference %d", list, ref_id);
  for (int k = 0; k < 3; k++)
    if (p[k].log2_denom > 7) return fail(FME_E_INVALID, "fme_set_wp: log2 denominator %d", (int)p[k].log2_denom);
  if (!c->wp_init) {
    for (auto& l : c->h_wp)
      for (auto& q : l)
        for (auto& r : q) r = fme_wp_param{1, 0, 0, {0, 0, 0}};
    c->wp_init = true;
  }
  for (int k = 0; k < 3; k++) c->h_wp[list][ref_id][k] = p[k];
  c->wp_dirty = true;
  return FME_OK;
}

int fme_mc_last_ms(fme_ctx* c, float* ms) {
  if (!c || !ms) return fail(FME_E_INVALID, "fme_mc_last_ms: null argument");
  if (!c->mc_timed) return fail(FME_E_STATE, "fme_mc_last_ms: no profiled motion compensation");
  HIP_TRY(hipEventSynchronize(c->ev_mc[1]));
  HIP_TRY(hipEventElapsedTime(ms, c->ev_mc[0], c->ev_mc[1]));
  return FME_OK;
}

int fme_set_profiling(fme_ctx* c, int enable) {
  if (!c) return fail(FME_E_INVALID, "fme_set_profiling: null ctx");
  HIP_TRY(hipSetDevice(c->device));
  if (enable && !c->events_made) {
    for (auto& set : c->ev)
      for (auto& e : set) HIP_TRY(hipEventCreate(&e));
    c->events_made = true;
  }
  if (!enable) FME_TRY(harvest_events(c, true));
  c->profiling = enable != 0;
  return FME_OK;
}

int fme_last_timings(fme_ctx* c, float* ms, int count) {
  if (!c || !ms || count < 0) return fail(FME_E_INVALID, "fme_last_timings: null argument");
  HIP_TRY(hipSetDevice(c->device));
  FME_TRY(harvest_events(c, true));
  if (!c->timed) return fail(FME_E_STATE, "fme_last_timings: no profiled batch");
  for (int i = 0; i < count && i < FME_NUM_TIMINGS; i++) ms[i] = c->last_ms[i];
  return FME_OK;
}

int fme_accumulated_timings(fme_ctx* c, double* ms, int count, int reset) {
  if (!c || (count > 0 && !ms) || count < 0) return fail(FME_E_INVALID, "fme_accumulated_timings: null argument");
  HIP_TRY(hipSetDevice(c->device));
  FME_TRY(harvest_events(c, true));
  const int n = c->acc_batches;
  for (int i = 0; i < count && i < FME_NUM_TIMINGS; i++) ms[i] = c->acc_ms[i];
  if (reset) {
    for (double& v : c->acc_ms) v = 0.0;
    c->acc_batches = 0;
  }
  return n;
}

}
```

hm16.9-nn_fme_amd/csrc/fme_ctx.h:

```cpp
#pragma once

#include <hip/hip_runtime.h>

#include <algorithm>
#include <cstdlib>
#include <cstring>
#include <string>
#include <thread>
#include <vector>

#include "fme_device.h"

namespace fme {

int fail(int code, const char* fmt, ...);

#define HIP_TRY(expr)                                                                            \
  do {                                                                                           \
    hipError_t _e = (expr);                                                                      \
    if (_e != hipSuccess)                                                                        \
      return fme::fail(_e == hipErrorOutOfMemory ? FME_E_NOMEM : FME_E_DEVICE, "%s: %s (%s:%d)", \
                       #expr, hipGetErrorString(_e), __FILE__, __LINE__);                        \
  } while (0)

#define FME_TRY(expr)           \
  do {                          \
    const int _rc = (expr);     \
    if (_rc) return _rc;        \
  } while (0)

template <typename T, bool kPinned>
struct Buf {
  T* p = nullptr;
  size_t cap = 0;
  hipError_t reserve(size_t n) {
    if (n <= cap) return hipSuccess;
    release();
    const size_t want = std::max<size_t>(kPinned ? n + n / 4 : n, 1);
    void** const pp = reinterpret_cast<void**>(&p);
    hipError_t e = kPinned ? hipHostMalloc(pp, want * sizeof(T), hipHostMallocDefault) : hipMalloc(pp, want * sizeof(T));
    if (e == hipSuccess) cap = kPinned ? want : n;
    return e;
  }
  void release() {
    if (p) (void)(kPinned ? hipHostFree(p) : hipFree(p));
    p = nullptr;
    cap = 0;
  }
};
template <typename T> using DevBuf = Buf<T, false>;
template <typename T> using HostBuf = Buf<T, true>;

template <typename F>
void par_for(int n, F&& f) {
  const unsigned hc = std::thread::hardware_concurrency();
  const int nt = n < 32768 ? 1 : (int)std::min<unsigned>(8u, hc ? hc : 1u);
  if (nt <= 1) {
    f(0, n);
    return;
  }
  std::vector<std::thread> th;
  th.reserve((size_t)nt - 1);
  for (int t = 1; t < nt; t++)
    th.emplace_back([&f, n, nt, t] { f((int)((long long)n * t / nt), (int)((long long)n * (t + 1) / nt)); });
  f(0, (int)((long long)n / nt));
  for (auto& x : th) x.join();
}
}

struct SingleStage {
  int32_t nn_out[4];
  uint32_t flag;
};

struct fme_ctx {
  int device = 0;
  fme_config cfg{};
  fme::PicDesc pics[FME_MAX_PICTURES]{};
  bool pic_owned[FME_MAX_PICTURES]{};
  size_t pic_bytes[FME_MAX_PICTURES]{};
  double mlambda[FME_MAX_LAMBDAS]{};
  bool lambda_set[FME_MAX_LAMBDAS]{};
  bool tables_dirty = true;

  fme::DevBuf<fme::PicDesc> d_pics;
  fme::DevBuf<double> d_mlambda;
  static constexpr int kTabSlots = 16;
  fme::TablesSlot* h_tab = nullptr;
  fme::TablesSlot* h_tab_dev = nullptr;
  hipEvent_t tab_ev[kTabSlots] = {};
  bool tab_used[kTabSlots] = {};
  int tab_next = 0;
  fme::DevBuf<int16_t> d_keys;
  size_t n_keys = 0;
  fme::DevBuf<float> d_nn;
  bool nn_loaded = false;
  fme_nn_net net{};
  fme::DevBuf<uint8_t> d_net;
  bool net_loaded = false;
  int nn_engine = FME_NN_ENGINE_EXACT;
  float* nn_margin = nullptr;
  int nn_margin_cap = 0;
  void* nn_logits = nullptr;
  int nn_logits_cap = 0;
  const uint32_t* nn_in = nullptr;
  int nn_in_cap = 0;

  fme::DevBuf<fme_job> d_jobs;
  fme::DevBuf<fme_result> d_res;
  fme::DevBuf<fme_mv_result> d_mv;
  fme::DevBuf<int32_t> koff;
  fme::DevBuf<uint8_t> cls;
  fme::DevBuf<int32_t> perm;
  fme::DevBuf<int32_t> counts;
  int counts_cur = 0;
  bool counts_dirty = false;
  fme::DevBuf<int32_t> blk_agg;
  fme::DevBuf<int32_t> blk_prefix;
  fme::DevBuf<uint32_t> nn_state;
  int state_cur = 0;
  bool state_pending = false;
  uint32_t pending_state[12] = {};
  fme::DevBuf<fme::Schedule> d_sched;
  fme::SchedParams sched_p{};
  int32_t* h_counts = nullptr;

  uint8_t* chroma_owned[FME_MAX_PICTURES]{};
  size_t chroma_bytes[FME_MAX_PICTURES]{};
  fme::DevBuf<fme_mc_job> d_mc_jobs;
  fme::DevBuf<uint8_t> d_mc_planes;
  fme::DevBuf<int32_t> d_mc_invalid;
  fme_wp_param h_wp[2][FME_MAX_PICTURES][3] = {};
  bool wp_init = false, wp_dirty = true;
  fme::DevBuf<fme_wp_param> d_mc_wp;
  hipEvent_t ev_mc[2] = {nullptr, nullptr};
  bool mc_timed = false;
  fme::DevBuf<fme_pe_task> d_pe_tasks;
  fme::DevBuf<uint32_t> d_pe_dist;
  fme::DevBuf<int32_t> d_pe_invalid;
  std::vector<fme_pe_task> h_pe_tasks;
  std::vector<uint32_t> h_pe_dist;
  hipStream_t pe_stream = nullptr;
  hipEvent_t ev_pe[2] = {nullptr, nullptr};
  bool pe_timed = false;
  fme::DevBuf<fme_sse_task> d_sse_tasks;
  fme::DevBuf<uint32_t> d_sse_out;
  fme::DevBuf<int32_t> d_sse_invalid;
  std::vector<fme_sse_task> h_sse_tasks;
  std::vector<uint32_t> h_sse_out;
  hipStream_t sse_stream = nullptr;
  hipEvent_t ev_sse[2] = {nullptr, nullptr};
  bool sse_timed = false;
  fme::DevBuf<fme_job> d_surf_jobs;
  fme::DevBuf<uint8_t> d_surf_probe;
  fme::DevBuf<fme_surface> d_surf_out;
  fme::DevBuf<fme_surface_pick> d_surf_pick;
  fme::DevBuf<int32_t> d_surf_invalid;
  hipStream_t surf_stream = nullptr;
  hipEvent_t ev_surf[2] = {nullptr, nullptr};
  bool surf_timed = false;
  fme::DevBuf<fme_tz_ext> d_tz_ext;
  fme::DevBuf<uint32_t> d_tz_sad;
  fme::DevBuf<uint32_t> d_tz_nn_in;
  hipEvent_t ev_tz[2] = {nullptr, nullptr};
  bool tz_timed = false;
  double pi_ms[FME_PI_PHASES] = {};
  int16_t int_mv_2n[2][FME_MAX_REFS][2] = {};
  fme::DevBuf<fme::AmvpTask> d_amvp;
  fme::DevBuf<int16_t> d_tz_emi;
  fme::DevBuf<uint32_t> d_amvp_sad;
  fme::DevBuf<fme::BiKeyTask> d_bikey;
  fme::DevBuf<int32_t> d_key_invalid;
  fme::DevBuf<int32_t> d_ch_i32;
  fme::DevBuf<int32_t> d_tzp;
  fme::DevBuf<int32_t> d_tzp_perm;
  fme::HostBuf<fme::AmvpTask> h_pi_tasks;
  fme::HostBuf<uint32_t> h_pi_tsad;
  fme::HostBuf<fme_job> h_pi_jobs;
  fme::HostBuf<fme_tz_ext> h_pi_ext;
  fme::HostBuf<int32_t> h_pi_idx;
  fme::HostBuf<int32_t> h_pi_psrc;
  fme::HostBuf<fme_mv_result> h_pi_mv;
  fme::HostBuf<fme_result> h_pi_last;
  fme::HostBuf<fme_result> h_pi_ures;
  fme::HostBuf<fme_job> h_pi_seq;
  fme::HostBuf<fme_mv_result> h_pi_rs;
  fme::HostBuf<uint32_t> h_pi_rows;
  std::vector<int> pi_base, pi_task, pi_src, pi_lvl, pi_start, pi_byarea;
  std::vector<int32_t> pi_off, pi_fill;
  std::vector<uint8_t> pi_amvp_idx;
  fme::DevBuf<fme_job> d_pi_jobs;
  fme::DevBuf<fme_tz_ext> d_pi_ext;
  fme::DevBuf<int32_t> d_pi_idx;

  struct SingleStage* stage = nullptr;
  uint8_t* stage_dev = nullptr;
  hipStream_t single_stream = nullptr;
  uint32_t single_seq = 0;
  fme::SrvBox* box = nullptr;
  fme::SrvBox* box_dev = nullptr;
  hipStream_t srv_stream = nullptr;
  bool srv_running = false;
  bool srv_orphan = false;
  static constexpr int kMaxStreams = 8;
  hipStream_t used_streams[kMaxStreams] = {};
  int n_used_streams = 0;
  bool used_overflow = false;
  uint32_t srv_epoch = 0;
  uint32_t srv_done = 0;
  uint32_t srv_nn_gen = 0;
  uint32_t nn_gen = 0;
  uint64_t srv_khz = 100000;
  bool srv_marks = false;

  static constexpr int kEv = 9;
  static constexpr int kEvSets = 32;
  bool profiling = false;
  bool events_made = false;
  hipEvent_t ev[kEvSets][kEv] = {};
  long long ev_head = 0;
  long long ev_tail = 0;
  bool timed = false;
  hipEvent_t ev_done = nullptr;
  hipEvent_t ev_search = nullptr;
  int search_reserve = 0;
  bool main10_px = false;
  bool batch_issued = false;
  float last_ms[FME_NUM_TIMINGS] = {};
  double acc_ms[FME_NUM_TIMINGS] = {};
  int acc_batches = 0;

  hipStream_t aux = nullptr;
  hipStream_t aux2 = nullptr;
  hipEvent_t ev_join2 = nullptr;
  hipEvent_t ev_fork = nullptr, ev_join = nullptr;
};

namespace fme {
size_t nn_deep_packed_bytes(const fme_nn_net& n);
void nn_deep_pack(const fme_nn_net& n, const double* params, void* out);
hipError_t launch_nn_deep_tail(const fme_nn_net& n, const void* packed, float* margin, void* logits, const BatchArgs& a,
                               const WorkBufs& w, int state_in, int engine, hipStream_t s);
hipError_t launch_nn_deep_single(const fme_nn_net& n, const void* packed, const NnIn11& in11, int32_t* out,
                                 uint32_t* flag, uint32_t seq, hipStream_t s);

int sync_tables(fme_ctx* c, hipStream_t s);
int grow_keys(fme_ctx* c, size_t n);
BatchArgs batch_args(const fme_ctx* c, const fme_job* jobs, int n);
int refine_batch(fme_ctx* c, const fme_job* d_jobs, fme_result* d_res, fme_mv_result* d_mv, int n, hipStream_t s,
                 const fme_job_packed* d_pjobs = nullptr, const int32_t* d_key_base = nullptr);
int tz_run(fme_ctx* c, fme_job* d_jobs, const fme_tz_ext* d_ext, uint32_t* d_sad, int n, void* stream, int16_t* d_emi,
           uint32_t* d_nn_in = nullptr, int ext_stride = (int)sizeof(fme_tz_ext));
int check_rejected(fme_ctx* c, hipStream_t s, const char* name, const char* what);
}
```

hm16.9-nn_fme_amd/nnfme/pipeline.py:

```python
import ctypes
import sys
import time

import numpy as np

from . import dist as fdist
from .abi import JOB_DTYPE, MV_RESULT_DTYPE

_hip = None


def _hip_lib():
    global _hip
    if _hip is None:
        h = ctypes.CDLL("libamdhip64.so.7")
        h.hipMemcpyAsync.argtypes = [ctypes.c_void_p, ctypes.c_void_p, ctypes.c_size_t, ctypes.c_int, ctypes.c_void_p]
        h.hipMemcpyAsync.restype = ctypes.c_int
        h.hipEventCreateWithFlags.argtypes = [ctypes.POINTER(ctypes.c_void_p), ctypes.c_uint]
        h.hipEventCreateWithFlags.restype = ctypes.c_int
        h.hipEventDestroy.argtypes = [ctypes.c_void_p]
        h.hipEventDestroy.restype = ctypes.c_int
        h.hipStreamWaitEvent.argtypes = [ctypes.c_void_p, ctypes.c_void_p, ctypes.c_uint]
        h.hipStreamWaitEvent.restype = ctypes.c_int
        _hip = h
    return _hip


SLOW_CALLS = []


def _memcpy_async(dst, src, nbytes, kind, stream):
    t0 = time.perf_counter()
    rc = _hip_lib().hipMemcpyAsync(dst.data_ptr(), src.data_ptr(), nbytes, kind, stream.cuda_stream)
    dt = (time.perf_counter() - t0) * 1e3
    if dt > 1.0:
        SLOW_CALLS.append(("hipMemcpyAsync kind %d" % kind, int(nbytes), round(dt, 3)))
    if rc != 0:
        raise RuntimeError(f"hipMemcpyAsync failed ({rc})")


def _timed(what, f):
    t0 = time.perf_counter()
    f()
    dt = (time.perf_counter() - t0) * 1e3
    if dt > 1.0:
        SLOW_CALLS.append((what, 0, round(dt, 3)))


class _RawEvent:

    def __init__(self):
        ev = ctypes.c_void_p()
        if _hip_lib().hipEventCreateWithFlags(ctypes.byref(ev), 2) != 0:
            raise RuntimeError("hipEventCreateWithFlags failed")
        self.cuda_event = ev.value

    def wait(self, stream):
        if _hip_lib().hipStreamWaitEvent(stream.cuda_stream, self.cuda_event, 0) != 0:
            raise RuntimeError("hipStreamWaitEvent failed")

    def destroy(self):
        if self.cuda_event and _hip is not None:
            _hip.hipEventDestroy(self.cuda_event)
        self.cuda_event = None

    def __del__(self):
        if sys.is_finalizing() or not self.cuda_event or _hip is None:
            return
        try:
            _hip.hipEventDestroy(self.cuda_event)
        except Exception:
            pass


H2D, D2H = 1, 2
D2D_NOCU = 1024


def torch_current_stream(t):
    import torch
    return torch.cuda.current_stream(t.device)


ORG0 = 32
REFS = 4


def group_jobs(base, frames, key_count=0):
    out = []
    for j in range(frames):
        g = np.array(base, dtype=JOB_DTYPE, copy=True)
        g["org_id"] = ORG0 + j
        g["ref_id"] = j + 3 - base["ref_id"].astype(np.int64)
        g["lambda_id"] = j
        bi = g["key_offset"] >= 0
        g["key_offset"][bi] += j * key_count
        out.append(g)
    return np.concatenate(out)


def group_key_reqs(base, frames, key_count):
    from .abi import BIKEY_REQ_DTYPE
    out = []
    for j in range(frames):
        g = np.array(base, dtype=BIKEY_REQ_DTYPE, copy=True)
        g["org_id"] = ORG0 + j
        g["ref_id"] = j + 3 - base["ref_id"].astype(np.int64)
        g["key_offset"] += j * key_count
        out.append(g)
    return np.concatenate(out)


class FrameReplay:
    def __init__(self, ctx, base_jobs, pool, lambda_of, n_steps, frames_per_step=1, world=1, rank=0, device=None,
                 group=None, defer_download=True, key_reqs=None, key_count=0, nn_rows=None,
                 download_engine="sdma", download_wgs=8, search_reserve=0, packed=True, copy_streams=1, slots=3,
                 max_ahead=4, precreate_events=True, warm_engines=True, timeline=False):
        import torch
        from .abi import JOB_PACKED_DTYPE
        from .runtime import FmeError, pack_jobs
        self.torch, self.ctx = torch, ctx
        self.world, self.rank, self.group = world, rank, group
        self.F = F = frames_per_step
        self.R = R = int(slots)
        if R < 2:
            raise ValueError("slots >= 2")
        self.lambda_of = lambda_of
        self.steps = n_steps
        P, H, W = pool.shape
        self.P, self.H, self.W = P, H, W
        if pool.dtype not in (np.uint8, np.uint16):
            raise ValueError(f"frame pool dtype {pool.dtype}: uint8 or uint16 (main10) samples")
        self.bps = pool.dtype.itemsize
        pdt = torch.uint8 if self.bps == 1 else torch.int16
        host = np.ascontiguousarray(pool).view(np.uint8 if self.bps == 1 else np.int16)
        self.pool = torch.from_numpy(host).pin_memory()
        self.key_count = int(key_count)
        self.jobs = group_jobs(base_jobs, F, self.key_count)
        self.n = n = len(self.jobs)
        self.packed, self.packed_reason = bool(packed), None
        if self.packed:
            try:
                pk, kb = pack_jobs(self.jobs)
            except FmeError as e:
                self.packed, self.packed_reason = False, str(e)
        if self.packed:
            self.h_jobs = torch.from_numpy(pk.view(np.uint8).copy()).pin_memory()
            self.h_kb = torch.from_numpy(kb.view(np.uint8).copy()).pin_memory()
            self.d_kb = [torch.empty(self.h_kb.numel(), dtype=torch.uint8, device=device) for _ in range(R)]
            assert self.h_jobs.numel() == n * JOB_PACKED_DTYPE.itemsize
        else:
            self.h_jobs = torch.from_numpy(self.jobs.view(np.uint8).copy()).pin_memory()
        self.job_bytes = self.h_jobs.numel() + (self.h_kb.numel() if self.packed else 0)
        self.d_jobs = [torch.empty(self.h_jobs.numel(), dtype=torch.uint8, device=device) for _ in range(R)]
        self.kreqs = None
        if key_reqs is not None and len(key_reqs):
            self.kreqs = group_key_reqs(key_reqs, F, self.key_count)
            self.h_kreqs = torch.from_numpy(self.kreqs.view(np.uint8).copy()).pin_memory()
            self.d_kreqs = [torch.empty(self.h_kreqs.numel(), dtype=torch.uint8, device=device) for _ in range(R)]
        self.rows = None
        if nn_rows is not None:
            self.rows = np.tile(np.ascontiguousarray(nn_rows, dtype=np.uint32).reshape(-1, 9), (F, 1))
            assert len(self.rows) == n
            self.h_rows = torch.from_numpy(self.rows.view(np.uint8).copy()).pin_memory()
            self.d_rows = [torch.empty(self.h_rows.numel(), dtype=torch.uint8, device=device) for _ in range(R)]
        self.d_out = [torch.empty(n * MV_RESULT_DTYPE.itemsize, dtype=torch.uint8, device=device) for _ in range(R)]
        self.h_out = torch.empty((n_steps, n * MV_RESULT_DTYPE.itemsize), dtype=torch.uint8).pin_memory()
        frames = n_steps * world * F
        self.recon = torch.empty((frames + REFS, H, W), dtype=pdt, device=device)
        self.org = torch.empty((n_steps * F, H, W), dtype=pdt, device=device)
        self.states = torch.zeros((n_steps, 12), dtype=torch.int32, device=device)
        self.s_comp = torch.cuda.default_stream(device)
        self.s_copy = torch.cuda.Stream(device)
        if copy_streams not in (1, 2):
            raise ValueError("copy_streams 1 or 2")
        self.copy_streams = copy_streams
        self.s_down = self.s_copy if copy_streams == 1 else torch.cuda.Stream(device)
        self.uploaded = -1
        self.ev_in = [torch.cuda.Event() for _ in range(n_steps)]
        self.ev_comp = [torch.cuda.Event() for _ in range(n_steps)]
        self.ev_out = [torch.cuda.Event() for _ in range(n_steps)]
        self.ev_search = [_RawEvent() for _ in range(n_steps)]
        if precreate_events:
            for e in self.ev_in + self.ev_comp + self.ev_out:
                e.record(self.s_copy)
            self.s_copy.synchronize()
        self.defer_download = defer_download
        if download_engine not in ("kernel", "blit", "sdma"):
            raise ValueError(f"download_engine {download_engine!r}")
        self.download_engine, self.download_wgs = download_engine, int(download_wgs)
        ctx.set_search_reserve(int(search_reserve))
        ctx.set_search_event(None)
        self.pending = None
        self.fixed_jobs = 0
        self.last_prefix = 0
        self.r_out = {}
        self.max_ahead = int(max_ahead)
        self.host_ms = []
        self.host_seg = []
        self.host_seg_names = ("upload", "waits", "bind", "refine", "prefetch", "download")
        self.warm_engines = bool(warm_engines)
        self.engines_warmed = None
        self.tl = None
        if timeline:
            self.tl = {kk: [torch.cuda.Event(enable_timing=True) for _ in range(n_steps)]
                       for kk in ("up0", "up1", "b0", "b1", "d0", "d1")}
            self.tl_base = torch.cuda.Event(enable_timing=True)

    def h2d_bytes_per_step(self):
        b = self.job_bytes + 2 * self.F * self.H * self.W * self.bps
        if self.kreqs is not None:
            b += self.h_kreqs.numel()
        if self.rows is not None:
            b += self.h_rows.numel()
        return b

    def close(self):
        try:
            self.ctx.set_search_event(None)
        except Exception:
            pass
        for e in self.ev_search:
            e.destroy()
        self.ev_search = []

    def first_frame(self, k):
        return (k * self.world + self.rank) * self.F

    def _publish(self, g, src_rank):
        dst = self.recon[g + REFS]
        if self.rank == src_rank:
            _memcpy_async(dst, self.pool[g % self.P], self.H * self.W * self.bps, H2D, torch_current_stream(dst))
        if self.world > 1:
            import torch.distributed as dist
            if dist.get_backend(self.group) == "gloo":
                tmp = dst.cpu()
                dist.broadcast(tmp, src=src_rank, group=self.group)
                dst.copy_(tmp, non_blocking=False)
            else:
                dist.broadcast(dst, src=src_rank, group=self.group)

    def rank_of_frame(self, g):
        return (g // self.F) % self.world

    def readers(self, h):
        frames = self.steps * self.world * self.F
        out = []
        for d in range(1, REFS + 1):
            f = h + d
            if 0 <= f < frames:
                r = self.rank_of_frame(f)
                if r not in out:
                    out.append(r)
        return out

    def _exchange(self, k, stream):
        import torch.distributed as dist
        F, W = self.F, self.world
        base = k * W * F
        gloo = dist.get_backend(self.group) == "gloo"
        ops, fixups = [], []
        for r in range(W):
            for j in range(F):
                h = base + r * F - 1 + j
                dsts = [d for d in self.readers(h) if d != r]
                if self.rank == r:
                    buf = self.recon[h + REFS]
                    if gloo:
                        stream.synchronize()
                        buf = buf.cpu()
                    for d in dsts:
                        ops.append(dist.P2POp(dist.isend, buf, d, group=self.group))
                elif self.rank in dsts:
                    buf = self.recon[h + REFS]
                    if gloo:
                        tmp = self.torch.empty_like(buf, device="cpu")
                        fixups.append((buf, tmp))
                        buf = tmp
                    ops.append(dist.P2POp(dist.irecv, buf, r, group=self.group))
        if ops:
            for w in dist.batch_isend_irecv(ops):
                w.wait()
        for dst, tmp in fixups:
            dst.copy_(tmp, non_blocking=False)

    def _upload_run(self, dst, d0, g0, count, stream):
        i = 0
        while i < count:
            s = (g0 + i) % self.P
            run = min(count - i, self.P - s)
            _memcpy_async(dst[d0 + i], self.pool[s], run * self.H * self.W * self.bps, H2D, stream)
            i += run

    def _publish_run(self, g0, count, src_rank, stream):
        if self.rank == src_rank:
            self._upload_run(self.recon, g0 + REFS, g0, count, stream)

    def prime(self):
        if self.warm_engines:
            self.engines_warmed = self.ctx.warm_copy_engines()
        with self.torch.cuda.stream(self.s_copy):
            for g in range(-REFS, -1):
                self._publish(g, 0)
        for k in range(self.steps):
            self._copy_down(k, self.s_down)
        self.s_copy.synchronize()
        self.s_down.synchronize()

    def _refine(self, k, out_ptr, n, stream):
        b = k % self.R
        if self.packed:
            self.ctx.refine_mv_packed_device(self.d_jobs[b].data_ptr(), self.d_kb[b].data_ptr(), out_ptr, n,
                                             stream.cuda_stream)
        else:
            self.ctx.refine_mv_device(self.d_jobs[b].data_ptr(), out_ptr, n, stream.cuda_stream)

    def bind_rows(self, b):
        if self.rows is not None:
            self.ctx.set_nn_inputs(self.d_rows[b].data_ptr(), self.n)

    def _bind(self, k):
        ctx, W, H, F = self.ctx, self.W, self.H, self.F
        self.bind_rows(k % self.R)
        f0 = self.first_frame(k)
        for j in range(F):
            ctx.bind_picture_device(ORG0 + j, self.org[k * F + j].data_ptr(), W, W, H)
            ctx.set_lambda(j, self.lambda_of(f0 + j))
        for s in range(F + REFS - 1):
            ctx.bind_picture_device(s, self.recon[f0 - REFS + s + REFS].data_ptr(), W, W, H)

    def _upload(self, k):
        F, R = self.F, self.R
        b = k % R
        f0 = self.first_frame(k)
        cp = self.s_copy
        with self.torch.cuda.stream(cp):
            if k >= R:
                _timed("copy stream wait_event", lambda: cp.wait_event(self.ev_comp[k - R]))
            if self.tl:
                self.tl["up0"][k].record(cp)
            _memcpy_async(self.d_jobs[b], self.h_jobs, self.h_jobs.numel(), H2D, cp)
            if self.packed:
                _memcpy_async(self.d_kb[b], self.h_kb, self.h_kb.numel(), H2D, cp)
            if self.rows is not None:
                _memcpy_async(self.d_rows[b], self.h_rows, self.h_rows.numel(), H2D, cp)
            if self.kreqs is not None:
                _memcpy_async(self.d_kreqs[b], self.h_kreqs, self.h_kreqs.numel(), H2D, cp)
            self._upload_run(self.org, k * F, f0, F, cp)
            base = k * self.world * F
            self._publish_run(base + self.rank * F - 1, F, self.rank, cp)
            if self.world > 1:
                self._exchange(k, cp)
            if self.tl:
                self.tl["up1"][k].record(cp)
            _timed("ev_in record", lambda: self.ev_in[k].record(cp))
        self.uploaded = k

    def issue(self, k, prefetch=True):
        pc = time.perf_counter
        t = [pc()]
        ctx = self.ctx
        b = k % self.R
        if self.max_ahead > 0 and k >= self.max_ahead:
            self.ev_comp[k - self.max_ahead].synchronize()
        if self.uploaded < k:
            self._upload(k)
        t.append(pc())
        comp = self.s_comp
        comp.wait_event(self.ev_in[k])
        if k >= self.R:
            comp.wait_event(self.ev_out[k - self.R])
        t.append(pc())
        self._bind(k)
        if self.kreqs is not None:
            ctx.build_bipred_keys_device(self.d_kreqs[b].data_ptr(), len(self.kreqs), self.key_count * self.F,
                                         comp.cuda_stream)
        if self.world > 1:
            ctx.nn_reset()
        if self.defer_download:
            ctx.set_search_event(self.ev_search[k])
        t.append(pc())
        if self.tl:
            self.tl["b0"][k].record(comp)
        self._refine(k, self.d_out[b].data_ptr(), self.n, comp)
        if self.world > 1:
            ctx.nn_copy_state_device(self.states[k].data_ptr(), comp.cuda_stream)
        if self.tl:
            self.tl["b1"][k].record(comp)
        self.ev_comp[k].record(comp)
        t.append(pc())
        if prefetch and k + 1 < self.steps:
            self._upload(k + 1)
        t.append(pc())
        if not self.defer_download:
            self._download(k, self.ev_comp[k])
        else:
            if self.pending is not None:
                self._download(self.pending, self.ev_search[k] if self.n > 0 else self.ev_comp[self.pending])
            self.pending = k
        t.append(pc())
        self.host_ms.append((t[-1] - t[0]) * 1e3)
        self.host_seg.append([round((t[i + 1] - t[i]) * 1e3, 3) for i in range(len(t) - 1)])

    def _copy_down(self, k, dn):
        b = k % self.R
        if self.download_engine == "kernel":
            self.ctx.download_device(self.d_out[b].data_ptr(), self.h_out[k].data_ptr(), self.h_out.shape[1],
                                     self.download_wgs, dn.cuda_stream)
        elif self.download_engine == "sdma":
            _memcpy_async(self.h_out[k], self.d_out[b], self.h_out.shape[1], D2D_NOCU, dn)
        else:
            _memcpy_async(self.h_out[k], self.d_out[b], self.h_out.shape[1], D2H, dn)

    def _download(self, k, after):
        dn = self.s_down
        if isinstance(after, _RawEvent):
            after.wait(dn)
        else:
            dn.wait_event(after)
        if self.tl:
            self.tl["d0"][k].record(dn)
        self._copy_down(k, dn)
        if self.tl:
            self.tl["d1"][k].record(dn)
        self.ev_out[k].record(dn)

    def drain(self):
        if self.pending is not None:
            self._download(self.pending, self.ev_comp[self.pending])
            self.pending = None
        self.s_copy.synchronize()
        self.s_comp.synchronize()
        self.s_down.synchronize()
        self.ctx.set_search_event(None)

    def check_status(self, first_step=0):
        from .abi import RES_REJECTED
        for k in range(first_step, self.steps):
            if np.any(self.results(k)["status"] & RES_REJECTED):
                raise RuntimeError(f"frame replay: step {k}'s batch was rejected on the device")

    def timeline_start(self):
        if self.tl:
            self.tl_base.record(self.s_comp)

    def timeline_rows(self, k0, k1):
        rows = []
        for k in range(k0, k1):
            r = {"step": k}
            for kk in ("up0", "up1", "b0", "b1", "d0", "d1"):
                r[kk] = round(self.tl_base.elapsed_time(self.tl[kk][k]), 4)
            rows.append(r)
        return rows

    def results(self, k):
        return self.h_out[k].numpy().view(MV_RESULT_DTYPE)

    def resident_outputs(self, k0, k1):
        torch = self.torch
        dev = self.d_out[0].device
        self.r_out = {k: torch.empty(self.n * MV_RESULT_DTYPE.itemsize, dtype=torch.uint8, device=dev)
                      for k in range(k0, k1)}

    def _resident_batch(self, k, n):
        ctx, comp = self.ctx, self.s_comp
        b = k % self.R
        self._bind(k)
        if self.kreqs is not None:
            ctx.build_bipred_keys_device(self.d_kreqs[b].data_ptr(), len(self.kreqs), self.key_count * self.F,
                                         comp.cuda_stream)
        self._refine(k, self.r_out[k].data_ptr(), n, comp)

    def issue_resident(self, k):
        ctx, comp = self.ctx, self.s_comp
        ctx.set_search_event(None)
        if self.world > 1:
            ctx.nn_reset()
        self._resident_batch(k, self.n)
        if self.world > 1:
            ctx.nn_copy_state_device(self.states[k].data_ptr(), comp.cuda_stream)

    def finish_resident(self, k0, k1, prefix):
        if self.world == 1 or prefix <= 0:
            return 0
        import torch.distributed as dist
        torch = self.torch
        self.s_comp.synchronize()
        st = self.states if dist.get_backend(self.group) != "gloo" else self.states.cpu()
        gathered = [torch.zeros_like(st) for _ in range(self.world)]
        dist.all_gather(gathered, st, group=self.group)
        bs = np.zeros((self.steps * self.world, 12), np.uint32)
        for r in range(self.world):
            g = gathered[r].cpu().numpy().view(np.uint32)
            for k in range(self.steps):
                bs[k * self.world + r] = g[k]
        carries, _ = fdist.chain_states(bs)
        fixed = 0
        for k in range(k0, k1):
            carry = carries[k * self.world + self.rank]
            if not int(carry[11]):
                continue
            self.ctx.nn_set_state(carry)
            self._resident_batch(k, prefix)
            fixed += prefix
        return fixed

    def finish(self, first_step=0):
        torch = self.torch
        self.drain()
        if self.world == 1:
            return 0
        import torch.distributed as dist
        st = self.states if dist.get_backend(self.group) != "gloo" else self.states.cpu()
        gathered = [torch.zeros_like(st) for _ in range(self.world)]
        dist.all_gather(gathered, st, group=self.group)
        bs = np.zeros((self.steps * self.world, 12), np.uint32)
        for r in range(self.world):
            g = gathered[r].cpu().numpy().view(np.uint32)
            for k in range(self.steps):
                bs[k * self.world + r] = g[k]
        carries, _ = fdist.chain_states(bs)
        fixed = 0
        ctx, comp = self.ctx, self.s_comp
        for k in range(first_step, self.steps):
            out = self.results(k)
            p = fdist.uninit_prefix(out)
            self.last_prefix = max(self.last_prefix, p)
            carry = carries[k * self.world + self.rank]
            if p == 0 or not int(carry[11]):
                continue
            with torch.cuda.stream(comp):
                self._bind(k)
                if self.kreqs is not None:
                    ctx.build_bipred_keys(self.kreqs, self.key_count * self.F, comp.cuda_stream)
                ctx.nn_set_state(carry)
                out[:p] = ctx.refine_mv(self.jobs[:p], comp.cuda_stream)
            fixed += p
        self.fixed_jobs = fixed
        return fixed
```

include/fme.h:

```cpp
#ifndef FME_H
#define FME_H

#include <stddef.h>
#include <stdint.h>

#ifdef __cplusplus
extern "C" {
#endif

#define FME_ABI_VERSION 18

#define FME_OK            0
#define FME_E_INVALID    -1
#define FME_E_DEVICE     -2
#define FME_E_NOMEM      -3
#define FME_E_UNSUPPORTED -4
#define FME_E_STATE      -5

#define FME_MAX_PICTURES  64
#define FME_MAX_LAMBDAS   64
#define FME_NN_PARAMS     2060

typedef struct fme_config {
  int32_t bit_depth;
  int32_t use_hadamard;
  int32_t nn_mode;
  int32_t qp;
  int32_t fast_inter_mode;
  int32_t max_jobs;
} fme_config;

#define FME_JOB_EMI       0x01u
#define FME_JOB_BIPRED    0x02u
#define FME_JOB_LOSSLESS  0x04u
#define FME_JOB_NN_IN     0x08u

typedef struct fme_job {
  uint16_t x, y;
  uint8_t  w, h;
  uint8_t  org_id, ref_id;
  int16_t  mv_x, mv_y;
  int16_t  mvp_x, mvp_y;
  int16_t  lt_x, lt_y, rb_x, rb_y;
  uint8_t  flags;
  uint8_t  lambda_id;
  uint16_t bits_in;
  int32_t  key_offset;
} fme_job;

#define FME_RES_NN_STALE   0x01u
#define FME_RES_NN_UNINIT  0x02u
#define FME_RES_REJECTED   0x8000u

typedef struct fme_result {
  int16_t  mv_int_x, mv_int_y;
  int16_t  mv_x, mv_y;
  int8_t   half_x, half_y, qtr_x, qtr_y;
  uint32_t frac_cost;
  uint32_t cost;
  uint32_t bits;
  uint32_t c;
  uint32_t emi[8];
  uint8_t  n_emi;
  uint8_t  nn_class;
  uint16_t status;
} fme_result;

typedef struct fme_mv_result {
  int16_t  mv_x, mv_y;
  uint32_t cost;
  uint32_t bits;
  uint8_t  nn_class;
  uint8_t  reserved;
  uint16_t status;
} fme_mv_result;

#define FME_PACK_WAVE        64
#define FME_PK_RANGE_TOP     0x1u
#define FME_PK_RANGE_BOTTOM  0x2u
#define FME_PK_RANGE_LEFT    0x4u
#define FME_PK_RANGE_RIGHT   0x8u
typedef struct fme_job_packed {
  uint32_t pu;
  uint32_t ctl;
  int16_t  mv_x, mv_y;
  int16_t  mvp_x, mvp_y;
} fme_job_packed;

typedef struct fme_ctx fme_ctx;

int         fme_abi_version(void);
int         fme_create(int device, const fme_config* cfg, fme_ctx** out_ctx);
int         fme_destroy(fme_ctx* ctx);
const char* fme_last_error(void);

int fme_set_picture(fme_ctx* ctx, int id, const uint8_t* luma, int stride, int width, int height,
                    void* stream);
int fme_bind_picture_device(fme_ctx* ctx, int id, const uint8_t* d_luma, int stride, int width,
                            int height);

int fme_set_picture_chroma(fme_ctx* ctx, int id, const uint8_t* cb, const uint8_t* cr, int stride,
                           void* stream);
int fme_bind_picture_chroma_device(fme_ctx* ctx, int id, const uint8_t* d_cb, const uint8_t* d_cr,
                                   int stride);

int fme_set_lambda(fme_ctx* ctx, int lambda_id, double lambda);
int fme_set_motion_lambda(fme_ctx* ctx, int lambda_id, double motion_lambda);

int fme_set_keys(fme_ctx* ctx, const int16_t* keys, size_t count, void* stream);

int fme_load_nn_weights(fme_ctx* ctx, const float* params, int count);
#define FME_NN_MAX_HIDDEN  4
#define FME_NN_MAX_WIDTH   40
#define FME_NN_F32         0
#define FME_NN_F64         1
#define FME_NN_EMB_NONE    0
#define FME_NN_EMB_MASTER  1
#define FME_NN_EMB_SWAP    2
#define FME_NN_OUT_LINEAR  0
#define FME_NN_OUT_SIGMOID 1
#define FME_NN_ENGINE_EXACT 0
#define FME_NN_ENGINE_MFMA  1

typedef struct fme_nn_net {
  int32_t  precision;
  int32_t  n_hidden;
  int32_t  width[FME_NN_MAX_HIDDEN];
  int32_t  embedding;
  int32_t  out_act;
  uint32_t carry_hidden;
  uint32_t input_flags;
} fme_nn_net;
#define FME_NN_IN_SLOT_RESET 1u
#define FME_NN_IN_TZ_RING    2u

int fme_set_nn_inputs(fme_ctx* ctx, const uint32_t* d_rows, int capacity);

int fme_nn_param_count(const fme_nn_net* net);
int fme_load_nn_net(fme_ctx* ctx, const fme_nn_net* net, const double* params, int count);
int fme_set_nn_engine(fme_ctx* ctx, int engine);
int fme_set_nn_margin_output(fme_ctx* ctx, float* d_margin, int capacity);
int fme_set_nn_logit_output(fme_ctx* ctx, void* d_logits, int capacity);

int fme_nn_reset_state(fme_ctx* ctx);
int fme_nn_get_state(fme_ctx* ctx, uint32_t* out12);
int fme_nn_set_state(fme_ctx* ctx, const uint32_t* in12);
int fme_nn_copy_state_device(fme_ctx* ctx, uint32_t* d_out12, void* stream);

int fme_set_search_event(fme_ctx* ctx, void* event);

int fme_set_search_reserve(fme_ctx* ctx, int workgroups);

int fme_download_device(fme_ctx* ctx, const void* d_src, void* h_dst, size_t bytes, int workgroups,
                        void* stream);

int fme_warm_copy_engines(fme_ctx* ctx, int* engines);


int fme_refine(fme_ctx* ctx, const fme_job* jobs, fme_result* results, int n, void* stream);
int fme_refine_device(fme_ctx* ctx, const fme_job* d_jobs, fme_result* d_results, int n,
                      void* stream);
int fme_refine_mv(fme_ctx* ctx, const fme_job* jobs, fme_mv_result* out, int n, void* stream);
int fme_refine_mv_device(fme_ctx* ctx, const fme_job* d_jobs, fme_mv_result* d_out, int n,
                         void* stream);
int fme_pack_jobs(const fme_job* jobs, int n, fme_job_packed* out, int32_t* key_base);
int fme_unpack_jobs(const fme_job_packed* packed, const int32_t* key_base, int n, fme_job* out);
int fme_refine_packed_device(fme_ctx* ctx, const fme_job_packed* d_jobs, const int32_t* d_key_base,
                             fme_result* d_results, int n, void* stream);
int fme_refine_mv_packed_device(fme_ctx* ctx, const fme_job_packed* d_jobs, const int32_t* d_key_base,
                                fme_mv_result* d_out, int n, void* stream);
int fme_refine_status(fme_ctx* ctx);

#define FME_TZ_PRED2NX2N 0x01u
#define FME_TZ_RING      0x02u
#define FME_TZ_FULL      0x04u
#define FME_TZ_ENHANCED  0x08u

typedef struct fme_tz_ext {
  uint16_t cu_x, cu_y;
  int16_t  pred2n_x, pred2n_y;
  uint8_t  flags;
  uint8_t  search_range;
  uint16_t reserved;
} fme_tz_ext;

typedef struct fme_tz_ext2 {
  fme_tz_ext base;
  int16_t    preds[3][2];
} fme_tz_ext2;

int fme_integer_search(fme_ctx* ctx, fme_job* jobs, const fme_tz_ext* ext, uint32_t* sad, int n,
                       void* stream);
int fme_integer_search2(fme_ctx* ctx, fme_job* jobs, const fme_tz_ext2* ext, uint32_t* sad, int n,
                        void* stream);
int fme_integer_search2_device(fme_ctx* ctx, fme_job* d_jobs, const fme_tz_ext2* d_ext, uint32_t* d_sad,
                               int n, void* stream);
int fme_integer_search_device(fme_ctx* ctx, fme_job* d_jobs, const fme_tz_ext* d_ext, uint32_t* d_sad,
                              int n, void* stream);
int fme_integer_search_ring(fme_ctx* ctx, fme_job* jobs, const fme_tz_ext* ext, uint32_t* sad,
                            uint32_t* nn_in, int n, void* stream);
int fme_integer_search_ring_device(fme_ctx* ctx, fme_job* d_jobs, const fme_tz_ext* d_ext,
                                   uint32_t* d_sad, uint32_t* d_nn_in, int n, void* stream);
int fme_integer_search_last_ms(fme_ctx* ctx, float* ms);

#define FME_MAX_REFS     4
#define FME_PU_LOSSLESS  0x01u
#define FME_PART_2Nx2N 0
#define FME_PART_2NxN  1
#define FME_PART_Nx2N  2
#define FME_PART_NxN   3
#define FME_PART_2NxnU 4
#define FME_PART_2NxnD 5
#define FME_PART_nLx2N 6
#define FME_PART_nRx2N 7

typedef struct fme_pu_req {
  uint16_t x, y;
  uint8_t  w, h;
  uint16_t cu_x, cu_y;
  uint8_t  part_size;
  uint8_t  depth;
  uint8_t  org_id;
  uint8_t  num_refs;
  uint8_t  ref_id[FME_MAX_REFS];
  uint8_t  n_cand[FME_MAX_REFS];
  int16_t  cand[FME_MAX_REFS][2][2];
  uint8_t  lambda_id;
  uint8_t  search_range;
  uint8_t  flags;
  uint8_t  reserved;
  uint16_t reserved2[3];
} fme_pu_req;

typedef struct fme_pu_res {
  int16_t  mv_x, mv_y;
  int16_t  mvp_x, mvp_y;
  uint8_t  ref_idx;
  uint8_t  mvp_idx;
  uint16_t reserved;
  uint32_t bits, cost;
  uint32_t ref_cost[FME_MAX_REFS];
  uint32_t ref_bits[FME_MAX_REFS];
  int16_t  ref_mv[FME_MAX_REFS][2];
  uint8_t  ref_mvp_idx[FME_MAX_REFS];
  uint32_t reserved2[2];
} fme_pu_res;

int fme_pred_inter_p(fme_ctx* ctx, const fme_pu_req* reqs, fme_pu_res* res, int n, void* stream);
int fme_pred_inter_reset(fme_ctx* ctx);
int fme_template_costs(fme_ctx* ctx, const fme_pu_req* reqs, uint32_t* costs, int n, void* stream);

#define FME_PU_FAST_ME_GEN_B 0x02u
#define FME_PU_CLIP_BIPRED   0x04u
#define FME_PU_MVD_L1_ZERO   0x08u

typedef struct fme_pu_req_b {
  uint16_t x, y;
  uint8_t  w, h;
  uint16_t cu_x, cu_y;
  uint8_t  part_size;
  uint8_t  depth;
  uint8_t  org_id;
  uint8_t  part_idx;
  uint8_t  cu_w;
  uint8_t  lambda_id;
  uint8_t  search_range;
  uint8_t  bipred_range;
  uint8_t  flags;
  uint8_t  num_refs[2];
  uint8_t  ref_id[2][FME_MAX_REFS];
  uint8_t  n_cand[2][FME_MAX_REFS];
  int8_t   l1_to_l0[FME_MAX_REFS];
  uint8_t  reserved[7];
  int16_t  cand[2][FME_MAX_REFS][2][2];
} fme_pu_req_b;

typedef struct fme_pu_res_b {
  uint8_t  inter_dir;
  uint8_t  ref_idx[2];
  uint8_t  mvp_idx[2];
  uint8_t  bi_list;
  uint8_t  bi_iters;
  uint8_t  reserved;
  int16_t  mv[2][2];
  int16_t  mvp[2][2];
  uint32_t bits, cost;
  uint32_t uni_cost[2];
  uint32_t uni_bits[2];
  uint32_t bi_cost, bi_bits;
  uint32_t ref_cost[2][FME_MAX_REFS];
  int16_t  ref_mv[2][FME_MAX_REFS][2];
  uint32_t bi_ref_cost[FME_MAX_REFS];
  int16_t  bi_ref_mv[FME_MAX_REFS][2];
  uint8_t  ref_mvp_idx[2][FME_MAX_REFS];
} fme_pu_res_b;

typedef struct fme_bikey_req {
  uint16_t x, y;
  uint8_t  w, h, org_id, ref_id;
  uint16_t cu_x, cu_y;
  int16_t  mv_x, mv_y;
  int32_t  key_offset;
  uint32_t flags;
} fme_bikey_req;
int fme_build_bipred_keys(fme_ctx* ctx, const fme_bikey_req* reqs, int n, size_t key_count, void* stream);
int fme_build_bipred_keys_device(fme_ctx* ctx, const fme_bikey_req* d_reqs, int n, size_t key_count,
                                 void* stream);

int fme_pred_inter_b(fme_ctx* ctx, const fme_pu_req_b* reqs, fme_pu_res_b* res, int n, void* stream);

#define FME_PI_PHASES 8
int fme_pred_inter_phases(fme_ctx* ctx, double* ms, int count);

int fme_frac_dif_single(fme_ctx* ctx, int lossless, const int16_t* key, int key_stride, int w,
                        int h, const int16_t* ref, int ref_stride, int mv_int_x, int mv_int_y,
                        int mvp_x, int mvp_y, double motion_lambda, int16_t* half_xy,
                        int16_t* qtr_xy, uint32_t* cost);

int fme_nn_pred_single(fme_ctx* ctx, const uint32_t* e, uint32_t c, int pu_h, int pu_w,
                       int* nn_class, int16_t* out4);

#define FME_MC_L0 0x01u
#define FME_MC_L1 0x02u
#define FME_MC_WP 0x04u

typedef struct fme_mc_job {
  uint16_t x, y;
  uint8_t  w, h;
  uint8_t  flags;
  uint8_t  reserved;
  uint8_t  ref_id[2];
  uint16_t cu_x, cu_y;
  int16_t  mv[2][2];
  uint16_t reserved2;
} fme_mc_job;

int fme_motion_compensate(fme_ctx* ctx, const fme_mc_job* jobs, int n, uint8_t* y, int y_stride,
                          uint8_t* cb, uint8_t* cr, int c_stride, int width, int height, void* stream);
int fme_motion_compensate_device(fme_ctx* ctx, const fme_mc_job* d_jobs, int n, uint8_t* d_y,
                                 int y_stride, uint8_t* d_cb, uint8_t* d_cr, int c_stride, int width,
                                 int height, void* stream);
int fme_mc_invalid_count(fme_ctx* ctx);
typedef struct fme_wp_param {
  int16_t weight;
  int16_t offset;
  uint8_t log2_denom;
  uint8_t reserved[3];
} fme_wp_param;
int fme_set_wp(fme_ctx* ctx, int list, int ref_id, const fme_wp_param* ycbcr);
int fme_mc_last_ms(fme_ctx* ctx, float* ms);

#define FME_NUM_TIMINGS 7
int fme_set_profiling(fme_ctx* ctx, int enable);
int fme_search_kernel_of_shape(int width, int height);
int fme_last_timings(fme_ctx* ctx, float* ms, int count);
int fme_accumulated_timings(fme_ctx* ctx, double* ms, int count, int reset);
int fme_single_last_device_us(fme_ctx* ctx, float* us, int count);

#ifdef __cplusplus
}
#endif

#endif
```

Before: 839.1 million.

## Double-buffer per-batch work buffers and alternate batches across two compute streams

Duplicates the per-batch scratch state (class/perm/scan buffers, key offsets, schedule, pic/lambda tables, result records) into two slots and rotates four counter blocks, so consecutive refine batches no longer share buffers. The Python pipeline alternates batches across two compute streams. Cross-stream ordering is kept with a ring of done events, and only the NN-state tail waits on the previous batch, so one batch's front/search can overlap the previous batch's tail. This adds event bookkeeping, more device memory, and a serial fallback whenever keys, deep NN, growth or foreign batches are involved.

```diff
diff --git a/hm16.9-nn_fme_amd/csrc/fme_api.cpp b/hm16.9-nn_fme_amd/csrc/fme_api.cpp
--- a/hm16.9-nn_fme_amd/csrc/fme_api.cpp
+++ b/hm16.9-nn_fme_amd/csrc/fme_api.cpp
@@ -47,18 +47,19 @@
   std::unique_ptr<fme_ctx> c(new fme_ctx());
   c->device = device;
   c->cfg = *cfg;
-  HIP_TRY(c->d_pics.reserve(FME_MAX_PICTURES));
-  HIP_TRY(c->d_mlambda.reserve(FME_MAX_LAMBDAS));
+  HIP_TRY(c->d_pics.reserve(kOvSlots * FME_MAX_PICTURES));
+  HIP_TRY(c->d_mlambda.reserve(kOvSlots * FME_MAX_LAMBDAS));
   HIP_TRY(c->d_nn.reserve(kNnPkFloats));
-  HIP_TRY(c->counts.reserve(2 * kCountWords));
-  HIP_TRY(hipMemset(c->counts.p, 0, 2 * kCountWords * sizeof(int32_t)));
-  HIP_TRY(c->d_sched.reserve(1));
+  HIP_TRY(c->counts.reserve(kOvBlocks * kCountWords));
+  HIP_TRY(hipMemset(c->counts.p, 0, kOvBlocks * kCountWords * sizeof(int32_t)));
+  HIP_TRY(c->d_sched.reserve(kOvSlots));
+  HIP_TRY(hipMemset(c->d_sched.p, 0, kOvSlots * sizeof(Schedule)));
+  for (auto& e : c->done_ev) HIP_TRY(hipEventCreateWithFlags(&e, hipEventDisableTiming));
   c->sched_p = sched_params();
   {
     const char* m10 = std::getenv("FME_MAIN10_SEARCH");
     c->main10_px = m10 && std::strcmp(m10, "px") == 0;
   }
-  HIP_TRY(hipEventCreateWithFlags(&c->ev_done, hipEventDisableTiming));
   HIP_TRY(c->nn_state.reserve(24));
   HIP_TRY(hipMemset(c->nn_state.p, 0, 24 * sizeof(uint32_t)));
   HIP_TRY(c->d_key_invalid.reserve(1));
@@ -68,10 +69,12 @@
     const size_t n = (size_t)cfg->max_jobs;
     const size_t nb = (n + kJobsPerScanBlock - 1) / kJobsPerScanBlock;
     if (n * kNumClasses > (size_t)INT32_MAX) return fail(FME_E_INVALID, "fme_create: max_jobs %d", cfg->max_jobs);
-    HIP_TRY(c->cls.reserve(n));
-    HIP_TRY(c->perm.reserve(n * kNumClasses));
-    HIP_TRY(c->blk_agg.reserve(nb * 9));
-    HIP_TRY(c->blk_prefix.reserve(nb * 9));
+    for (int b = 0; b < kOvSlots; b++) {
+      HIP_TRY(c->cls[b].reserve(n));
+      HIP_TRY(c->perm[b].reserve(n * kNumClasses));
+      HIP_TRY(c->blk_agg[b].reserve(nb * 9));
+      HIP_TRY(c->blk_prefix[b].reserve(nb * 9));
+    }
   }
   *out_ctx = c.release();
   return FME_OK;
@@ -79,6 +82,16 @@
 
 }
 static int srv_stop(fme_ctx* c);
+static hipEvent_t done_event(const fme_ctx* c, int back) {
+  if (back < 1 || back > 2 || !c->ov.live[back - 1]) return nullptr;
+  return c->done_ev[(c->ov.seq - back) % fme_ctx::kDoneRing];
+}
+static int wait_batches(fme_ctx* c, hipStream_t s) {
+  for (int back = 1; back <= 2; back++)
+    if (hipEvent_t e = done_event(c, back))
+      if (c->ov.stream[back - 1] != s) HIP_TRY(hipStreamWaitEvent(s, e, 0));
+  return FME_OK;
+}
 static void note_stream(fme_ctx* c, hipStream_t s) {
   for (int i = 0; i < c->n_used_streams; i++)
     if (c->used_streams[i] == s) return;
@@ -94,6 +107,7 @@
   return FME_OK;
 }
 int fme::grow_keys(fme_ctx* c, size_t n) {
+  c->keys_fresh = true;
   if (n <= c->d_keys.cap) return FME_OK;
   FME_TRY(drain_ctx(c));
   HIP_TRY(c->d_keys.reserve(n));
@@ -131,10 +145,16 @@
   for (auto& e : c->ev_surf)
     if (e) (void)hipEventDestroy(e);
   c->d_pics.release(); c->d_mlambda.release(); c->d_keys.release(); c->d_nn.release(); c->d_net.release();
-  c->d_jobs.release(); c->d_res.release(); c->d_mv.release(); c->koff.release(); c->cls.release(); c->perm.release();
-  c->counts.release(); c->blk_agg.release(); c->blk_prefix.release(); c->nn_state.release();
+  c->d_jobs.release(); c->d_res.release(); c->d_res1.release(); c->d_mv.release();
+  for (int b = 0; b < kOvSlots; b++) {
+    c->koff[b].release(); c->cls[b].release(); c->perm[b].release(); c->blk_agg[b].release(); c->blk_prefix[b].release();
+  }
+  c->counts.release(); c->nn_state.release();
   c->d_sched.release();
-  if (c->ev_done) (void)hipEventDestroy(c->ev_done);
+  for (auto& e : c->done_ev)
+    if (e) (void)hipEventDestroy(e);
+  for (auto& e : c->state_read_ev)
+    if (e) (void)hipEventDestroy(e);
   if (c->stage) (void)hipHostFree(c->stage);
   if (c->single_stream) (void)hipStreamDestroy(c->single_stream);
   if (c->box) (void)hipHostFree(c->box);
@@ -271,6 +291,7 @@
   FME_TRY(srv_stop(c));
   FME_TRY(grow_keys(c, count));
   hipStream_t s = static_cast<hipStream_t>(stream);
+  FME_TRY(wait_batches(c, s));
   if (count) HIP_TRY(hipMemcpyAsync(c->d_keys.p, keys, count * sizeof(int16_t), hipMemcpyHostToDevice, s));
   HIP_TRY(hipMemsetAsync(c->d_key_invalid.p, 0, sizeof(int32_t), s));
   HIP_TRY(hipStreamSynchronize(s));
@@ -397,51 +418,51 @@
   if (!c || !d_out12) return fail(FME_E_INVALID, "fme_nn_copy_state_device: null argument");
   HIP_TRY(hipSetDevice(c->device));
   hipStream_t s = static_cast<hipStream_t>(stream);
-  if (c->state_pending)
+  if (c->state_pending) {
     HIP_TRY(launch_put_state(d_out12, c->pending_state, s));
-  else
-    HIP_TRY(hipMemcpyAsync(d_out12, c->nn_state.p + 12 * c->state_cur, 12 * sizeof(uint32_t),
-                           hipMemcpyDeviceToDevice, s));
-  return FME_OK;
-}
-
-}
-
-static int ensure_work(fme_ctx* c, int n) {
+    return FME_OK;
+  }
+  FME_TRY(wait_batches(c, s));
+  HIP_TRY(hipMemcpyAsync(d_out12, c->nn_state.p + 12 * c->state_cur, 12 * sizeof(uint32_t),
+                         hipMemcpyDeviceToDevice, s));
+  hipEvent_t& e = c->state_read_ev[c->state_reads++ % fme_ctx::kDoneRing];
+  if (!e) HIP_TRY(hipEventCreateWithFlags(&e, hipEventDisableTiming));
+  HIP_TRY(hipEventRecord(e, s));
+  c->state_read_last = e;
+  c->state_read_stream = s;
+  return FME_OK;
+}
+
+}
+
+static int ensure_work(fme_ctx* c, int n, bool* grows = nullptr) {
   const size_t nb = ((size_t)n + kJobsPerScanBlock - 1) / kJobsPerScanBlock;
   if ((size_t)n * kNumClasses > (size_t)INT32_MAX) return fail(FME_E_INVALID, "%d jobs in one batch", n);
-  HIP_TRY(c->cls.reserve(n));
-  HIP_TRY(c->perm.reserve((size_t)n * kNumClasses));
-  HIP_TRY(c->blk_agg.reserve(nb * 9));
-  HIP_TRY(c->blk_prefix.reserve(nb * 9));
-  HIP_TRY(c->koff.reserve(n));
-  return FME_OK;
-}
-
-static int counts_begin(fme_ctx* c, hipStream_t s) {
-  if (c->counts_dirty) HIP_TRY(hipMemsetAsync(c->counts.p, 0, 2 * kCountWords * sizeof(int32_t), s));
-  c->counts_dirty = true;
-  return FME_OK;
-}
-static void counts_done(fme_ctx* c) {
-  c->counts_cur ^= 1;
-  c->counts_dirty = false;
-}
-
-static WorkBufs work_bufs(fme_ctx* c) {
+  if (grows) *grows = (size_t)n > c->cls[0].cap || (size_t)n > c->koff[0].cap;
+  for (int b = 0; b < kOvSlots; b++) {
+    HIP_TRY(c->cls[b].reserve(n));
+    HIP_TRY(c->perm[b].reserve((size_t)n * kNumClasses));
+    HIP_TRY(c->blk_agg[b].reserve(nb * 9));
+    HIP_TRY(c->blk_prefix[b].reserve(nb * 9));
+    HIP_TRY(c->koff[b].reserve(n));
+  }
+  return FME_OK;
+}
+
+static WorkBufs work_bufs(fme_ctx* c, int slot, int block, int zeroed) {
   WorkBufs w{};
-  w.cls = c->cls.p;
-  w.perm = c->perm.p;
-  w.perm_cap = (int32_t)(c->perm.cap / kNumClasses);
-  w.koff = c->koff.p;
-  w.counts = c->counts.p + c->counts_cur * kCountWords;
-  w.counts_next = c->counts.p + (c->counts_cur ^ 1) * kCountWords;
+  w.cls = c->cls[slot].p;
+  w.perm = c->perm[slot].p;
+  w.perm_cap = (int32_t)(c->perm[slot].cap / kNumClasses);
+  w.koff = c->koff[slot].p;
+  w.counts = c->counts.p + block * kCountWords;
+  w.counts_next = c->counts.p + zeroed * kCountWords;
   w.cursor = w.counts + kCursorWord;
   w.tile_ctr = w.counts + kTileCtrWord;
-  w.blk_agg = c->blk_agg.p;
-  w.blk_prefix = c->blk_prefix.p;
+  w.blk_agg = c->blk_agg[slot].p;
+  w.blk_prefix = c->blk_prefix[slot].p;
   w.nn_state = c->nn_state.p;
-  w.sched = c->d_sched.p;
+  w.sched = c->d_sched.p + slot;
   w.mv_out = nullptr;
   return w;
 }
@@ -460,10 +481,14 @@
   return a;
 }
 
-int fme::sync_tables(fme_ctx* c, hipStream_t s) {
+static int put_tables(fme_ctx* c, int slot, hipStream_t s) {
   note_stream(c, s);
   FME_TRY(srv_stop(c));
-  if (!c->tables_dirty) return FME_OK;
+  if (c->tables_dirty) {
+    c->tab_gen++;
+    c->tables_dirty = false;
+  }
+  if (c->slot_gen[slot] == c->tab_gen) return FME_OK;
   if (!c->h_tab) {
     void* p = nullptr;
     HIP_TRY(hipHostMalloc(&p, fme_ctx::kTabSlots * sizeof(TablesSlot), hipHostMallocMapped));
@@ -478,10 +503,30 @@
   if (c->tab_used[k]) HIP_TRY(hipEventSynchronize(c->tab_ev[k]));
   std::memcpy(c->h_tab[k].pics, c->pics, sizeof(c->pics));
   std::memcpy(c->h_tab[k].ml, c->mlambda, sizeof(c->mlambda));
-  HIP_TRY(launch_put_tables(c->d_pics.p, c->d_mlambda.p, c->h_tab_dev + k, s));
+  HIP_TRY(launch_put_tables(c->d_pics.p + slot * FME_MAX_PICTURES, c->d_mlambda.p + slot * FME_MAX_LAMBDAS,
+                            c->h_tab_dev + k, s));
   HIP_TRY(hipEventRecord(c->tab_ev[k], s));
   c->tab_used[k] = true;
-  c->tables_dirty = false;
+  c->slot_gen[slot] = c->tab_gen;
+  return FME_OK;
+}
+
+int fme::sync_tables(fme_ctx* c, hipStream_t s) {
+  FME_TRY(wait_batches(c, s));
+  return put_tables(c, 0, s);
+}
+
+static int batch_begin(fme_ctx* c, const OverlapPlan& plan, hipStream_t s, hipEvent_t* done) {
+  hipEvent_t const prev_done = done_event(c, 1), slot_done = done_event(c, 2);
+  *done = c->done_ev[c->ov.seq % fme_ctx::kDoneRing];
+  if (c->ov.seq >= fme_ctx::kDoneRing)
+    HIP_TRY(hipEventSynchronize(c->done_ev[(c->ov.seq + 2) % fme_ctx::kDoneRing]));
+  if (plan.wait_prev_front) HIP_TRY(hipStreamWaitEvent(s, prev_done, 0));
+  if (plan.wait_slot) HIP_TRY(hipStreamWaitEvent(s, slot_done, 0));
+  if (plan.fill_blocks) {
+    FME_TRY(drain_ctx(c));
+    HIP_TRY(hipMemsetAsync(c->counts.p, 0, kOvBlocks * kCountWords * sizeof(int32_t), s));
+  }
   return FME_OK;
 }
 
@@ -528,19 +573,28 @@
   if (c->cfg.nn_mode == 2 && c->nn_logits && n > c->nn_logits_cap)
     return fail(FME_E_INVALID, "fme_refine: %d jobs but the logit output holds %d", n, c->nn_logits_cap);
   HIP_TRY(hipSetDevice(c->device));
-  FME_TRY(ensure_work(c, n));
-  FME_TRY(sync_tables(c, s));
-  FME_TRY(apply_pending_state(c, s));
+  bool grows = false;
+  FME_TRY(ensure_work(c, n, &grows));
+  const uint32_t features = (c->keys_fresh ? kOvKeys : 0u) | (c->cfg.nn_mode == 2 ? kOvDeepNn : 0u) |
+                            (c->cfg.bit_depth > 8 && c->main10_px ? kOvPx : 0u) |
+                            (d_jobs && d_jobs == c->d_jobs.p ? kOvStaged : 0u) | (grows ? kOvGrow : 0u);
+  const OverlapPlan plan = overlap_plan(c->ov, s, features);
+  hipEvent_t const prev_done = done_event(c, 1);
+  hipEvent_t done = nullptr;
+  FME_TRY(batch_begin(c, plan, s, &done));
+  FME_TRY(put_tables(c, plan.slot, s));
 
   BatchArgs a = batch_args(c, d_jobs, n);
+  a.pics = c->d_pics.p + plan.slot * FME_MAX_PICTURES;
+  a.mlambda = c->d_mlambda.p + plan.slot * FME_MAX_LAMBDAS;
   a.pjobs = d_jobs ? nullptr : d_pjobs;
   a.key_base = d_key_base;
-  a.koff = c->koff.p;
+  a.koff = c->koff[plan.slot].p;
   a.res = d_res;
   a.nn_mode = c->cfg.nn_mode ? 1 : 0;
   a.nn_in = c->nn_in;
   a.nn_in_cap = c->nn_in_cap;
-  WorkBufs w = work_bufs(c);
+  WorkBufs w = work_bufs(c, plan.slot, plan.block, plan.block_zeroed);
   w.mv_out = d_mv;
 
   const bool prof = c->profiling;
@@ -556,7 +610,7 @@
     ev = c->ev[eb];
     HIP_TRY(hipEventRecord(ev[0], s));
   }
-  FME_TRY(counts_begin(c, s));
+  overlap_begin(c->ov);
   HIP_TRY(launch_front(a, w, c->sched_p, s));
   if (prof) HIP_TRY(hipEventRecord(ev[3], s));
   if (c->ev_search) HIP_TRY(hipEventRecord(c->ev_search, s));
@@ -569,6 +623,12 @@
     HIP_TRY(launch_search_lane(a, w, c->search_reserve, s));
   }
   if (prof) HIP_TRY(hipEventRecord(ev[4], s));
+  if (plan.wait_prev_tail) HIP_TRY(hipStreamWaitEvent(s, prev_done, 0));
+  if (c->state_read_last) {
+    if (c->state_read_stream != s) HIP_TRY(hipStreamWaitEvent(s, c->state_read_last, 0));
+    c->state_read_last = nullptr;
+  }
+  FME_TRY(apply_pending_state(c, s));
   if (prof) HIP_TRY(hipEventRecord(ev[5], s));
   HIP_TRY(c->cfg.nn_mode == 2
               ? launch_nn_deep_tail(c->net, c->d_net.p, c->nn_margin, c->nn_logits, a, w, c->state_cur, c->nn_engine, s)
@@ -577,18 +637,28 @@
     HIP_TRY(hipEventRecord(ev[6], s));
     c->ev_head++;
   }
-  HIP_TRY(hipEventRecord(c->ev_done, s));
-  counts_done(c);
+  HIP_TRY(hipEventRecord(done, s));
+  c->ev_done = done;
+  c->last_slot = plan.slot;
+  c->keys_fresh = false;
+  overlap_commit(c->ov, s, features, plan);
   c->batch_issued = true;
   if (a.nn_mode) c->state_cur ^= 1;
   return FME_OK;
 }
 
 int fme::check_rejected(fme_ctx* c, hipStream_t s, const char* name, const char* what) {
-  HIP_TRY(hipMemcpyAsync(c->h_counts, &c->d_sched.p->invalid, sizeof(int32_t), hipMemcpyDeviceToHost, s));
+  HIP_TRY(hipMemcpyAsync(c->h_counts, &c->d_sched.p[c->last_slot].invalid, sizeof(int32_t), hipMemcpyDeviceToHost, s));
   HIP_TRY(hipStreamSynchronize(s));
   if (c->h_counts[0] > 0)
     return fail(FME_E_INVALID, "%s: %d job(s) %s", name, c->h_counts[0], what);
+  return FME_OK;
+}
+
+static int slot_records(fme_ctx* c, int n, fme_result** out) {
+  DevBuf<fme_result>& b = c->ov.seq % kOvSlots ? c->d_res1 : c->d_res;
+  HIP_TRY(b.reserve(n));
+  *out = b.p;
   return FME_OK;
 }
 
@@ -606,8 +676,9 @@
   if (n < 0) return fail(FME_E_INVALID, "fme_refine_mv_device: n = %d", n);
   if (n == 0) return FME_OK;
   HIP_TRY(hipSetDevice(c->device));
-  HIP_TRY(c->d_res.reserve(n));
-  return refine_batch(c, d_jobs, c->d_res.p, d_out, n, static_cast<hipStream_t>(stream));
+  fme_result* d_res = nullptr;
+  FME_TRY(slot_records(c, n, &d_res));
+  return refine_batch(c, d_jobs, d_res, d_out, n, static_cast<hipStream_t>(stream));
 }
 
 int fme_pack_jobs(const fme_job* jobs, int n, fme_job_packed* out, int32_t* key_base) {
@@ -696,10 +767,7 @@
   if (n < 0) return fail(FME_E_INVALID, "%s: n = %d", fn, n);
   if (n == 0) return FME_OK;
   HIP_TRY(hipSetDevice(c->device));
-  if (!d_res) {
-    HIP_TRY(c->d_res.reserve(n));
-    d_res = c->d_res.p;
-  }
+  if (!d_res) FME_TRY(slot_records(c, n, &d_res));
   return refine_batch(c, nullptr, d_res, d_mv, n, static_cast<hipStream_t>(stream), d_jobs, d_key_base);
 }
 
@@ -851,21 +919,21 @@
   HIP_TRY(hipSetDevice(c->device));
   HIP_TRY(hipEventSynchronize(c->ev_done));
   int32_t v = 0;
-  HIP_TRY(hipMemcpy(&v, &c->d_sched.p->invalid, sizeof(v), hipMemcpyDeviceToHost));
+  HIP_TRY(hipMemcpy(&v, &c->d_sched.p[c->last_slot].invalid, sizeof(v), hipMemcpyDeviceToHost));
   return v;
 }
 
 int fme_debug_front(fme_ctx* c, int32_t* perm_out, long long perm_words, int32_t* sched_out, int sched_words,
                     int32_t* cap_out) {
   if (!c || !c->batch_issued) return fail(FME_E_STATE, "fme_debug_front: no batch issued");
-  if (perm_words < 0 || (size_t)perm_words > c->perm.cap || sched_words < 0 ||
+  if (perm_words < 0 || (size_t)perm_words > c->perm[c->last_slot].cap || sched_words < 0 ||
       (size_t)sched_words * sizeof(int32_t) > sizeof(Schedule))
     return fail(FME_E_INVALID, "fme_debug_front: length");
   HIP_TRY(hipSetDevice(c->device));
   HIP_TRY(hipEventSynchronize(c->ev_done));
-  if (perm_out && perm_words) HIP_TRY(hipMemcpy(perm_out, c->perm.p, (size_t)perm_words * sizeof(int32_t), hipMemcpyDeviceToHost));
-  if (sched_out && sched_words) HIP_TRY(hipMemcpy(sched_out, c->d_sched.p, (size_t)sched_words * sizeof(int32_t), hipMemcpyDeviceToHost));
-  if (cap_out) *cap_out = (int32_t)(c->perm.cap / kNumClasses);
+  if (perm_out && perm_words) HIP_TRY(hipMemcpy(perm_out, c->perm[c->last_slot].p, (size_t)perm_words * sizeof(int32_t), hipMemcpyDeviceToHost));
+  if (sched_out && sched_words) HIP_TRY(hipMemcpy(sched_out, c->d_sched.p + c->last_slot, (size_t)sched_words * sizeof(int32_t), hipMemcpyDeviceToHost));
+  if (cap_out) *cap_out = (int32_t)(c->perm[c->last_slot].cap / kNumClasses);
   return FME_OK;
 }
 
@@ -883,15 +951,17 @@
   BatchArgs a = batch_args(c, d_jobs, n);
   a.nn_in = c->nn_in;
   a.nn_in_cap = c->nn_in_cap;
-  WorkBufs w = work_bufs(c);
+  const OverlapPlan plan = overlap_plan(c->ov, s, kOvForeign);
+  hipEvent_t done = nullptr;
+  FME_TRY(batch_begin(c, plan, s, &done));
+  WorkBufs w = work_bufs(c, plan.slot, plan.block, plan.block_zeroed);
   if (c->profiling) {
     if (!c->ev_tz[0]) {
       HIP_TRY(hipEventCreate(&c->ev_tz[0]));
       HIP_TRY(hipEventCreate(&c->ev_tz[1]));
     }
   }
-  c->counts_dirty = true;
-  HIP_TRY(hipMemsetAsync(w.counts, 0, kCountWords * sizeof(int32_t), s));
+  overlap_begin(c->ov);
   HIP_TRY(launch_classify(a, w, s));
   HIP_TRY(hipMemcpyAsync(c->h_counts, w.counts, kCountWords * sizeof(int32_t), hipMemcpyDeviceToHost, s));
   HIP_TRY(hipStreamSynchronize(s));
@@ -913,7 +983,7 @@
   HIP_TRY(launch_scatter(a, w, c->sched_p, s));
   TzArgs ta{};
   ta.a = a;
-  ta.perm = c->perm.p;
+  ta.perm = w.perm;
   ta.jobs_out = d_jobs;
   ta.ext = d_ext;
   ta.ext_stride = ext_stride;
@@ -975,6 +1045,8 @@
   HIP_TRY(hipStreamWaitEvent(s, c->ev_join2, 0));
   if (c->profiling) HIP_TRY(hipEventRecord(c->ev_tz[1], s));
   c->tz_timed = c->profiling;
+  HIP_TRY(hipEventRecord(done, s));
+  overlap_commit(c->ov, s, kOvForeign, plan);
   return FME_OK;
 }
 
diff --git a/hm16.9-nn_fme_amd/csrc/fme_ctx.h b/hm16.9-nn_fme_amd/csrc/fme_ctx.h
--- a/hm16.9-nn_fme_amd/csrc/fme_ctx.h
+++ b/hm16.9-nn_fme_amd/csrc/fme_ctx.h
@@ -10,6 +10,7 @@
 #include <vector>
 
 #include "fme_device.h"
+#include "fme_overlap_host.h"
 
 namespace fme {
 
@@ -85,6 +86,7 @@
 
   fme::DevBuf<fme::PicDesc> d_pics;
   fme::DevBuf<double> d_mlambda;
+  unsigned long long tab_gen = 1, slot_gen[fme::kOvSlots] = {};
   static constexpr int kTabSlots = 16;
   fme::TablesSlot* h_tab = nullptr;
   fme::TablesSlot* h_tab_dev = nullptr;
@@ -108,15 +110,23 @@
 
   fme::DevBuf<fme_job> d_jobs;
   fme::DevBuf<fme_result> d_res;
+  fme::DevBuf<fme_result> d_res1;
   fme::DevBuf<fme_mv_result> d_mv;
-  fme::DevBuf<int32_t> koff;
-  fme::DevBuf<uint8_t> cls;
-  fme::DevBuf<int32_t> perm;
+  fme::DevBuf<int32_t> koff[fme::kOvSlots];
+  fme::DevBuf<uint8_t> cls[fme::kOvSlots];
+  fme::DevBuf<int32_t> perm[fme::kOvSlots];
+  fme::DevBuf<int32_t> blk_agg[fme::kOvSlots];
+  fme::DevBuf<int32_t> blk_prefix[fme::kOvSlots];
   fme::DevBuf<int32_t> counts;
-  int counts_cur = 0;
-  bool counts_dirty = false;
-  fme::DevBuf<int32_t> blk_agg;
-  fme::DevBuf<int32_t> blk_prefix;
+  fme::OverlapState ov;
+  static constexpr int kDoneRing = 16;
+  hipEvent_t done_ev[kDoneRing] = {};
+  hipEvent_t state_read_ev[kDoneRing] = {};
+  long long state_reads = 0;
+  hipEvent_t state_read_last = nullptr;
+  hipStream_t state_read_stream = nullptr;
+  int last_slot = 0;
+  bool keys_fresh = false;
   fme::DevBuf<uint32_t> nn_state;
   int state_cur = 0;
   bool state_pending = false;
diff --git a/hm16.9-nn_fme_amd/csrc/fme_overlap_host.h b/hm16.9-nn_fme_amd/csrc/fme_overlap_host.h
--- /dev/null
+++ b/hm16.9-nn_fme_amd/csrc/fme_overlap_host.h
@@ -0,0 +1,66 @@
+#pragma once
+
+#include <cstdint>
+
+namespace fme {
+
+constexpr int kOvSlots = 2;
+constexpr int kOvBlocks = 4;
+
+enum : uint32_t {
+  kOvKeys = 1u << 0,
+  kOvDeepNn = 1u << 1,
+  kOvPx = 1u << 2,
+  kOvStaged = 1u << 3,
+  kOvGrow = 1u << 4,
+  kOvForeign = 1u << 5,
+  kOvFill = 1u << 6,
+};
+
+struct OverlapPlan {
+  int slot = 0;
+  int block = 0;
+  int block_zeroed = 0;
+  bool serial = false;
+  bool fill_blocks = false;
+  bool wait_slot = false;
+  bool wait_prev_front = false;
+  bool wait_prev_tail = false;
+};
+
+struct OverlapState {
+  long long seq = 0;
+  bool dirty = false;
+  const void* stream[2] = {nullptr, nullptr};
+  bool live[2] = {false, false};
+  uint32_t prev_features = 0;
+};
+
+inline OverlapPlan overlap_plan(const OverlapState& st, const void* stream, uint32_t features) {
+  OverlapPlan p;
+  p.slot = (int)(st.seq % kOvSlots);
+  p.block = (int)(st.seq % kOvBlocks);
+  p.block_zeroed = (int)((st.seq + 2) % kOvBlocks);
+  p.fill_blocks = st.dirty;
+  p.serial = features != 0 || st.dirty || st.prev_features != 0;
+  const bool other1 = st.live[0] && st.stream[0] != stream;
+  const bool other2 = st.live[1] && st.stream[1] != stream;
+  p.wait_slot = other2;
+  p.wait_prev_front = p.serial && other1;
+  p.wait_prev_tail = other1 && !p.wait_prev_front;
+  return p;
+}
+
+inline void overlap_begin(OverlapState& st) { st.dirty = true; }
+
+inline void overlap_commit(OverlapState& st, const void* stream, uint32_t features, const OverlapPlan& plan) {
+  st.seq++;
+  st.prev_features = features | (plan.fill_blocks ? (uint32_t)kOvFill : 0u);
+  st.dirty = false;
+  st.stream[1] = st.stream[0];
+  st.live[1] = st.live[0];
+  st.stream[0] = stream;
+  st.live[0] = true;
+}
+
+}
diff --git a/hm16.9-nn_fme_amd/nnfme/pipeline.py b/hm16.9-nn_fme_amd/nnfme/pipeline.py
--- a/hm16.9-nn_fme_amd/nnfme/pipeline.py
+++ b/hm16.9-nn_fme_amd/nnfme/pipeline.py
@@ -115,7 +115,7 @@
     def __init__(self, ctx, base_jobs, pool, lambda_of, n_steps, frames_per_step=1, world=1, rank=0, device=None,
                  group=None, defer_download=True, key_reqs=None, key_count=0, nn_rows=None,
                  download_engine="sdma", download_wgs=8, search_reserve=0, packed=True, copy_streams=1, slots=3,
-                 max_ahead=4, precreate_events=True, warm_engines=True, timeline=False):
+                 max_ahead=4, precreate_events=True, warm_engines=True, timeline=False, compute_streams=2):
         import torch
         from .abi import JOB_PACKED_DTYPE
         from .runtime import FmeError, pack_jobs
@@ -171,6 +171,10 @@
         self.org = torch.empty((n_steps * F, H, W), dtype=pdt, device=device)
         self.states = torch.zeros((n_steps, 12), dtype=torch.int32, device=device)
         self.s_comp = torch.cuda.default_stream(device)
+        if compute_streams not in (1, 2):
+            raise ValueError("compute_streams 1 or 2")
+        self.compute_streams = compute_streams
+        self.s_comps = [self.s_comp] + [torch.cuda.Stream(device) for _ in range(compute_streams - 1)]
         self.s_copy = torch.cuda.Stream(device)
         if copy_streams not in (1, 2):
             raise ValueError("copy_streams 1 or 2")
@@ -220,9 +224,14 @@
             self.ctx.set_search_event(None)
         except Exception:
             pass
+        for sc in self.s_comps:
+            sc.synchronize()
         for e in self.ev_search:
             e.destroy()
         self.ev_search = []
+
+    def comp_stream(self, k):
+        return self.s_comps[k % len(self.s_comps)]
 
     def first_frame(self, k):
         return (k * self.world + self.rank) * self.F
@@ -366,7 +375,7 @@
         if self.uploaded < k:
             self._upload(k)
         t.append(pc())
-        comp = self.s_comp
+        comp = self.comp_stream(k)
         comp.wait_event(self.ev_in[k])
         if k >= self.R:
             comp.wait_event(self.ev_out[k - self.R])
@@ -396,7 +405,7 @@
             self._download(k, self.ev_comp[k])
         else:
             if self.pending is not None:
-                self._download(self.pending, self.ev_search[k] if self.n > 0 else self.ev_comp[self.pending])
+                self._download(self.pending, self.ev_search[k] if self.n > 0 else None)
             self.pending = k
         t.append(pc())
         self.host_ms.append((t[-1] - t[0]) * 1e3)
@@ -416,8 +425,10 @@
         dn = self.s_down
         if isinstance(after, _RawEvent):
             after.wait(dn)
-        else:
+        elif after is not None:
             dn.wait_event(after)
+        if after is not self.ev_comp[k]:
+            dn.wait_event(self.ev_comp[k])
         if self.tl:
             self.tl["d0"][k].record(dn)
         self._copy_down(k, dn)
@@ -430,7 +441,8 @@
             self._download(self.pending, self.ev_comp[self.pending])
             self.pending = None
         self.s_copy.synchronize()
-        self.s_comp.synchronize()
+        for sc in self.s_comps:
+            sc.synchronize()
         self.s_down.synchronize()
         self.ctx.set_search_event(None)
 
@@ -463,7 +475,7 @@
                       for k in range(k0, k1)}
 
     def _resident_batch(self, k, n):
-        ctx, comp = self.ctx, self.s_comp
+        ctx, comp = self.ctx, self.comp_stream(k)
         b = k % self.R
         self._bind(k)
         if self.kreqs is not None:
@@ -472,7 +484,7 @@
         self._refine(k, self.r_out[k].data_ptr(), n, comp)
 
     def issue_resident(self, k):
-        ctx, comp = self.ctx, self.s_comp
+        ctx, comp = self.ctx, self.comp_stream(k)
         ctx.set_search_event(None)
         if self.world > 1:
             ctx.nn_reset()
@@ -485,7 +497,8 @@
             return 0
         import torch.distributed as dist
         torch = self.torch
-        self.s_comp.synchronize()
+        for sc in self.s_comps:
+            sc.synchronize()
         st = self.states if dist.get_backend(self.group) != "gloo" else self.states.cpu()
         gathered = [torch.zeros_like(st) for _ in range(self.world)]
         dist.all_gather(gathered, st, group=self.group)
diff --git a/include/fme.h b/include/fme.h
--- a/include/fme.h
+++ b/include/fme.h
@@ -148,6 +148,7 @@
 int fme_nn_copy_state_device(fme_ctx* ctx, uint32_t* d_out12, void* stream);
 
 int fme_set_search_event(fme_ctx* ctx, void* event);
+
 
 int fme_set_search_reserve(fme_ctx* ctx, int workgroups);
 
```

Result: faster. 916.5 million, median of 6 (+9.2%).
